# tmbdev/clstm

Hardware: AMD Instinct MI355X
Metric: text-line images/sec (fwd+bwd+CTC), 100-unit BiLSTM H=48 T~200 (higher is better)
Workload: dtype f32 (operand-exact split): forward, recurrences, CTC, decode in f32 arithmetic; the backward weight-gradient / softmax-backward products take their f32 operands split EXACTLY into three bf16 terms each (x1 + x2 + x3 = x) and sum the six bf16-MFMA products of weight >= 2^-16 in f32 -- what is dropped

## Files before the change

clstm_amd/csrc/dbgopt.h:

```cpp
#pragma once
#include <cstdlib>
#include <cstring>
#include <map>
#include <stdexcept>
#include <string>

namespace clstm {
struct DbgOptDef { const char* name; int dflt; };
inline constexpr DbgOptDef DBG_OPTS[] = {
    {"gemm_stag", 2},
    {"bwd_c32", 1},
    {"rec_x3", 1},
    {"pack_tiles", 1},
    {"fuse_wx", 1},
    {"gemm_b16mc", 1},
    {"dw_x3", 1},
    {"gemm_x3", 1},
    {"split_terms", 3},
    {"xd_prologue", 2},
    {"fwd_mfma", 1},
    {"bwd_mfma", 1},
    {"bwd_mfma_fused", 1},
    {"ctc_float", 0},
    {"peer_two_phase", 1},
};
inline const DbgOptDef* dbg_opt_def(const char* name) {
  for (const DbgOptDef& o : DBG_OPTS)
    if (strcmp(o.name, name) == 0) return &o;
  return nullptr;
}
inline std::map<std::string, int>& dbg_opts() {
  static std::map<std::string, int> m = [] {
    std::map<std::string, int> r;
    const char* e = getenv("CLSTM_DEBUG");
    if (e) {
      std::string s(e);
      size_t i = 0;
      while (i < s.size()) {
        size_t j = s.find(',', i);
        if (j == std::string::npos) j = s.size();
        const std::string kv = s.substr(i, j - i);
        const size_t eq = kv.find('=');
        if (!kv.empty()) {
          const std::string name = kv.substr(0, eq);
          if (eq == std::string::npos || !dbg_opt_def(name.c_str()))
            throw std::runtime_error("CLSTM_DEBUG: unknown option '" + name + "' (clstm_amd/csrc/dbgopt.h lists them as name=value)");
          r[name] = atoi(kv.c_str() + eq + 1);
        }
        i = j + 1;
      }
    }
    return r;
  }();
  return m;
}
inline int dbg_opt(const char* name) {
  const DbgOptDef* d = dbg_opt_def(name);
  if (!d) throw std::logic_error(std::string("internal: option '") + name + "' is not in DBG_OPTS");
  const auto& m = dbg_opts();
  const auto it = m.find(name);
  return it == m.end() ? d->dflt : it->second;
}
}
```

clstm_amd/csrc/devintrin.h:

```cpp
#pragma once

#ifdef CLSTM_HIP_EMU
#include "hip_emu.h"
#else
#include <hip/hip_runtime.h>
#include <hip/hip_ext.h>
#include <vector>

typedef float f32x4 __attribute__((ext_vector_type(4)));
typedef float f32x2 __attribute__((ext_vector_type(2)));
typedef unsigned u32x2 __attribute__((ext_vector_type(2)));

#define DEVFN __device__ __forceinline__
#define DEVMFN __device__ __forceinline__

template <int CTRL>
DEVFN float dpp_mov(float x) {
  const int xi = __builtin_bit_cast(int, x);
  return __builtin_bit_cast(float, __builtin_amdgcn_update_dpp(xi, xi, CTRL, 0xF, 0xF, false));
}
template <int CTRL>
DEVFN float dpp_perm(float x) {
  return __builtin_bit_cast(float, __builtin_amdgcn_update_dpp(0, __builtin_bit_cast(int, x), CTRL, 0xF, 0xF, true));
}
// ... 119 lines not shown
typedef unsigned u32x4 __attribute__((ext_vector_type(4)));
DEVFN u32x2 lds_read_tr16(const unsigned short* p) {
  return __builtin_bit_cast(u32x2, __builtin_amdgcn_ds_read_tr16_b64_v4i16((i16x4 __attribute__((address_space(3)))*)p));
}
typedef unsigned LdsAddr;
DEVFN LdsAddr lds_addr(const void* p) { return (unsigned)(size_t)(const __attribute__((address_space(3))) void*)p; }
DEVFN LdsAddr lds_addr_add(LdsAddr a, int bytes) { return a + (unsigned)bytes; }
template <int OFF>
DEVFN u32x2 lds_read_tr16_raw(LdsAddr addr) {
  u32x2 r;
  asm volatile("ds_read_b64_tr_b16 %0, %1 offset:%2" : "=v"(r) : "v"(addr), "n"(OFF));
  return r;
}
DEVFN u16x8 join_u16x8(u32x2 a, u32x2 b) {
  u32x4 v;
  v[0] = a[0]; v[1] = a[1]; v[2] = b[0]; v[3] = b[1];
  return __builtin_bit_cast(u16x8, v);
}

DEVFN int wave_uniform(int x) { return __builtin_amdgcn_readfirstlane(x); }
DEVFN long long dev_clock() { return (long long)__builtin_readcyclecounter(); }
DEVFN long long wall_clock() { return (long long)__builtin_amdgcn_s_memrealtime(); }
DEVFN float fast_exp(float x) { return __expf(x); }
DEVFN float fast_exp2(float x) { return __builtin_amdgcn_exp2f(x); }
DEVFN float fast_rcp(float x) { return __builtin_amdgcn_rcpf(x); }
DEVFN float fast_log2(float x) { return __builtin_amdgcn_logf(x); }

struct BufF32 { __amdgpu_buffer_rsrc_t r; };
constexpr unsigned BUF_OOB = 0xFFFFFFF0u;
constexpr unsigned BUF_OOB_BASE = 0x80000000u;
DEVFN BufF32 make_buf(const float* base, size_t bytes) {
  BufF32 b;
  b.r = __builtin_amdgcn_make_buffer_rsrc((void*)base, 0, (int)(bytes > 0x7FFFFFF0ull ? 0x7FFFFFF0ull : bytes), 0x00020000);
  return b;
}
DEVFN float buf_load(BufF32 b, unsigned byte_off) {
  return __builtin_bit_cast(float, __builtin_amdgcn_raw_buffer_load_b32(b.r, byte_off, 0, 0));
}
typedef int i32x4 __attribute__((ext_vector_type(4)));
typedef int i32x2 __attribute__((ext_vector_type(2)));
DEVFN f32x4 buf_load4(BufF32 b, unsigned byte_off) {
  return __builtin_bit_cast(f32x4, __builtin_amdgcn_raw_buffer_load_b128(b.r, byte_off, 0, 0));
}
DEVFN void buf_store(BufF32 b, unsigned byte_off, float v) {
  __builtin_amdgcn_raw_buffer_store_b32(__builtin_bit_cast(int, v), b.r, byte_off, 0, 0);
}
DEVFN void lds_dma16(BufF32 b, unsigned byte_off, void* lds_wave_base) {
  __builtin_amdgcn_raw_ptr_buffer_load_lds(b.r, (__attribute__((address_space(3))) void*)lds_wave_base, 16, byte_off, 0, 0, 0);
}
DEVFN void lds_dma4(BufF32 b, unsigned byte_off, void* lds_wave_base) {
  __builtin_amdgcn_raw_ptr_buffer_load_lds(b.r, (__attribute__((address_space(3))) void*)lds_wave_base, 4, byte_off, 0, 0, 0);
}
template <int N> DEVFN void wait_vmcnt() { asm volatile("s_waitcnt vmcnt(%0)" ::"n"(N) : "memory"); }
DEVFN void wait_lgkmcnt0() { asm volatile("s_waitcnt lgkmcnt(0)" ::: "memory"); }
DEVFN void wg_barrier() { __builtin_amdgcn_s_barrier(); }
DEVFN void wave_lds_fence() { __builtin_amdgcn_fence(__ATOMIC_ACQ_REL, "wavefront"); }
DEVFN float buf_load_s(BufF32 b, unsigned lane_off, unsigned uniform_off) {
  return __builtin_bit_cast(float, __builtin_amdgcn_raw_buffer_load_b32(b.r, lane_off, uniform_off, 0));
}
DEVFN void buf_store_s(BufF32 b, unsigned lane_off, unsigned uniform_off, float v) {
  __builtin_amdgcn_raw_buffer_store_b32(__builtin_bit_cast(int, v), b.r, lane_off, uniform_off, 0);
}
DEVFN void buf_store4(BufF32 b, unsigned byte_off, f32x4 v) {
  __builtin_amdgcn_raw_buffer_store_b128(__builtin_bit_cast(i32x4, v), b.r, byte_off, 0, 0);
}
DEVFN void buf_store_u32(BufF32 b, unsigned byte_off, unsigned v) { __builtin_amdgcn_raw_buffer_store_b32((int)v, b.r, byte_off, 0, 0); }
DEVFN void buf_store_u32x2_s(BufF32 b, unsigned lane_off, unsigned uniform_off, u32x2 v) {
  __builtin_amdgcn_raw_buffer_store_b64(__builtin_bit_cast(i32x2, v), b.r, lane_off, uniform_off, 0);
}
DEVFN void buf_store_u32_s(BufF32 b, unsigned lane_off, unsigned uniform_off, unsigned v) {
  __builtin_amdgcn_raw_buffer_store_b32((int)v, b.r, lane_off, uniform_off, 0);
}
DEVFN float max_f32(float x, float y) {
  float r;
  asm("v_max_f32 %0, %1, %2" : "=v"(r) : "v"(x), "v"(y));
  return r;
}

DEVFN f32x4 buf_load4_dev(BufF32 b, unsigned byte_off) {
  return __builtin_bit_cast(f32x4, __builtin_amdgcn_raw_buffer_load_b128(b.r, byte_off, 0, 16));
}
#define COMPILER_MEMORY_BARRIER() asm volatile("" ::: "memory")
DEVFN void buf_store_wt(BufF32 b, unsigned byte_off, float v) {
  __builtin_amdgcn_raw_buffer_store_b32(__builtin_bit_cast(int, v), b.r, byte_off, 0, 17);
}
DEVFN f32x4 buf_load4_wt(BufF32 b, unsigned byte_off) {
  return __builtin_bit_cast(f32x4, __builtin_amdgcn_raw_buffer_load_b128(b.r, byte_off, 0, 17));
}
DEVFN float buf_load_wt(BufF32 b, unsigned byte_off) {
  return __builtin_bit_cast(float, __builtin_amdgcn_raw_buffer_load_b32(b.r, byte_off, 0, 17));
}
DEVFN void buf_store4_wt(BufF32 b, unsigned byte_off, f32x4 v) {
  __builtin_amdgcn_raw_buffer_store_b128(__builtin_bit_cast(i32x4, v), b.r, byte_off, 0, 17);
}
DEVFN int load_i32_wt(const int* p) { return __hip_atomic_load(p, __ATOMIC_RELAXED, __HIP_MEMORY_SCOPE_SYSTEM); }
DEVFN void store_i32_wt(int* p, int v) { __hip_atomic_store(p, v, __ATOMIC_RELAXED, __HIP_MEMORY_SCOPE_SYSTEM); }
DEVFN void atomic_add_i32(int* p, int v) { atomicAdd(p, v); }
DEVFN int atomic_fetch_add_i32(int* p, int v) { return atomicAdd(p, v); }
DEVFN int hw_xcc_id() { unsigned x; asm volatile("s_getreg_b32 %0, hwreg(HW_REG_XCC_ID)" : "=s"(x)); return (int)(x & 0xF); }
DEVFN void sleep_some() { __builtin_amdgcn_s_sleep(16); }
DEVFN void poll_pause() { __builtin_amdgcn_s_sleep(1); }
DEVFN void sleep_iterations(int n) {
  n = n > 40 ? 40 : n;
  for (int i = 0; i < n; i++) __builtin_amdgcn_s_sleep(13);
}
DEVFN int wave_max_i(int x) {
#pragma unroll
  for (int m = 32; m >= 1; m >>= 1) { const int y = __shfl_xor(x, m, 64); x = y > x ? y : x; }
  return x;
}
DEVFN void drain_vmem() { asm volatile("s_waitcnt vmcnt(0)" ::: "memory"); }
DEVFN unsigned mad_u24(unsigned a, unsigned b, unsigned c) { return __umul24(a, b) + c; }
constexpr int GRID_WATCHDOG_SPINS = 1 << 21;
struct ClstmLaunchEvents { hipEvent_t a, b; };
inline thread_local std::vector<ClstmLaunchEvents>* clstm_launch_sink = nullptr;
inline thread_local std::vector<ClstmLaunchEvents> clstm_event_pool;
inline ClstmLaunchEvents clstm_launch_events() {
  ClstmLaunchEvents e{};
  if (!clstm_event_pool.empty()) { e = clstm_event_pool.back(); clstm_event_pool.pop_back(); }
  else { (void)hipEventCreate(&e.a); (void)hipEventCreate(&e.b); }
  clstm_launch_sink->push_back(e);
  return e;
}
#define CLSTM_LAUNCH_COOP(kernel, grid, block, smem, stream, argstruct)                                  \
  do {                                                                                                   \
    void* coop_args_[] = {(void*)&(argstruct)};                                                          \
    ClstmLaunchEvents ev_{};                                                                             \
    if (clstm_launch_sink) { ev_ = clstm_launch_events(); HIPCHECK(hipEventRecord(ev_.a, (hipStream_t)(stream))); } \
    HIPCHECK(hipLaunchCooperativeKernel((const void*)(kernel), grid, block, coop_args_, smem, (hipStream_t)(stream))); \
    if (ev_.b) HIPCHECK(hipEventRecord(ev_.b, (hipStream_t)(stream)));                                   \
  } while (0)

#define KEEP_ALIVE(x) asm volatile("" ::"v"(x))
#define SCHED_FENCE() __builtin_amdgcn_sched_barrier(0)
#define OPAQUE(x) asm volatile("" : "+v"(x))
#define KEEP_ALIVE2(x) asm volatile("" ::"v"(x))

template <typename T>
DEVFN T* dyn_smem() {
  extern __shared__ __attribute__((aligned(16))) char clstm_dyn_smem_[];
  return reinterpret_cast<T*>(clstm_dyn_smem_);
}

#define CLSTM_LAUNCH(kernel, grid, block, smem, stream, ...)                                                       \
  do {                                                                                                             \
    if (__builtin_expect(clstm_launch_sink != nullptr, 0)) {                                                       \
      const ClstmLaunchEvents ev_ = clstm_launch_events();                                                         \
      hipExtLaunchKernelGGL(kernel, grid, block, smem, (hipStream_t)(stream), ev_.a, ev_.b, 0, __VA_ARGS__);       \
    } else hipLaunchKernelGGL(kernel, grid, block, smem, (hipStream_t)(stream), __VA_ARGS__);                      \
  } while (0)
#endif

DEVFN bool dev_err_set(const int* err) { return err && (err[0] | err[1] | err[2] | err[3] | err[6] | err[7]) != 0; }
DEVFN bool f32_finite(float x) { return (__builtin_bit_cast(unsigned, x) & 0x7f800000u) != 0x7f800000u; }
DEVFN void raise_nonfinite(int* nanflag, int step_no) { if (*nanflag == 0) *nanflag = step_no; }


constexpr int PROG_STRIDE = 32;

constexpr int STAG_NA = 64, STAG_KA = 16;
__host__ __device__ inline constexpr bool stag_on(int nk4) { return nk4 >= 5; }
__host__ __device__ inline int stag_fwd_k(int q, int kk, int ku) { return kk < STAG_KA ? STAG_KA * q + kk : STAG_NA + (ku - STAG_KA) * q + (kk - STAG_KA); }
__host__ __device__ inline int stag_fwd_slot(int cell, int ku, int qs) {
  return cell < STAG_NA ? (cell / STAG_KA) * qs + (cell % STAG_KA)
                        : ((cell - STAG_NA) / (ku - STAG_KA)) * qs + STAG_KA + (cell - STAG_NA) % (ku - STAG_KA);
}

DEVFN float tanh_dev(float x) {
  const float xc = fminf(fmaxf(x, -15.0f), 15.0f);
  const float e = fast_exp(2.0f * xc);
  const float big = (e - 1.0f) * fast_rcp(e + 1.0f);
  const float small = xc - xc * xc * xc * (1.0f / 3.0f);
  return fabsf(xc) < 0.01f ? small : big;
}

DEVFN float sigmoid_dev(float x) { return fast_rcp(1.0f + fast_exp(-x)); }

DEVFN float gate_act(float x, bool is_tanh) {
  const float ax = fabsf(x);
  const unsigned mask = is_tanh ? 0x7FFFFFFFu : 0xFFFFFFFFu;
  const float scale = is_tanh ? -2.0f * 1.44269504088896341f : -1.44269504088896341f;
  const float e = fast_exp2(__builtin_bit_cast(float, __builtin_bit_cast(unsigned, x) & mask) * scale);
  const float r = fast_rcp(1.0f + e);
  const float s = ax * ax;
  const float p = fmaf(s, fmaf(s, fmaf(s, fmaf(s, fmaf(s, -1382.0f / 155925.0f, 62.0f / 2835.0f), -17.0f / 315.0f), 2.0f / 15.0f), -1.0f / 3.0f), 1.0f);
  const float th = copysignf(ax < 0.35f ? ax * p : (1.0f - e) * r, x);
  return is_tanh ? th : r;
}

constexpr float ACT_SIG_SCALE = -1.44269504088896341f, ACT_TANH_SCALE = -2.0f * 1.44269504088896341f;
DEVFN float act_affine(float x, float scale, float A, float B) {
  const float r = fast_rcp(1.0f + fast_exp2(x * scale));
  return fmaf(r, A, B);
}
DEVFN float tanh_fast(float x) { return act_affine(x, ACT_TANH_SCALE, 2.0f, -1.0f); }
```

clstm_amd/csrc/gemm_dw.h:

```cpp
#pragma once
#include <type_traits>
#include "gemm_bf16.h"

namespace clstm {

struct DwSlab {
  int tile_begin, ntiles;
  int need_it;
  int dir;
  int out_z;
  int pad[3];
};

struct XdArgs {
  GemmOperand A;
  GemmOperand B;
  float* out; int ld;
  int K;
  int* ready; int ready0;
};

struct GemmDwArgs {
  const float* S; long long sdir; int lds; long long s_elems;
  const float* D; int M; int no4; long long d_elems;
  const int* ktab;
  int ntiles_max;
  const DwSlab* slabs;
  int nslabs;
  const int* prog;
  const int* line_off;
  int bs, prog_base, ndir;
  float* partial;
  int R, Cn;
  unsigned gx, gy;
  int* timeouts;
  int* minprog;
  int tcap;
  int* done;
  int done_target;
  long long* trace;
  int trace_base;
  const float* xS; int xlds; long long xs_elems;
  const float* xD; int xM; long long xd_elems;
  const int* xtab; const DwSlab* xslabs; int xnslabs;
  float* xpartial; int xR, xCn; unsigned xgx, xgy;
  int x3;
  int terms;
  XdArgs xd;
};

constexpr int DW_PF = 3;
constexpr int DW_STAB_MAX = 256;
constexpr int dw_img_floats(int nt) { return nt <= 2 ? 8192 : 2 * 2 * nt * 64 * 32 / 2; }
constexpr int dw_smem_floats(int nt) { return dw_img_floats(nt) + 2 * DW_STAB_MAX; }
static_assert(8192 >= GEMM_BT * GEMM_LDO, "epilogue tile");

constexpr int DW_WATCHDOG_POLLS = 1 << 16;

DEVFN void gemm_dw_monitor(const GemmDwArgs& a) {
  if (threadIdx.x >= 64) return;
  const int lane = threadIdx.x & 63;
  int polls = 0;
  for (;;) {
    int all = 0x3fffffff;
    int pv[2][4];
#pragma unroll
    for (int dir = 0; dir < 2; dir++)
#pragma unroll
      for (int j = 0; j < 4; j++) {
        const int b = lane + 64 * j;
        pv[dir][j] = dir < a.ndir && b < a.bs ? load_i32_wt(a.prog + ((size_t)dir * a.bs + b) * PROG_STRIDE) : 0;
      }
    for (int dir = 0; dir < a.ndir; dir++) {
      int m = 0x3fffffff;
      for (int b = lane, j = 0; b < a.bs; b += 64, j++) {
        const int T = a.line_off[b + 1] - a.line_off[b];
        const int p = (j < 4 ? pv[dir][j] : load_i32_wt(a.prog + ((size_t)dir * a.bs + b) * PROG_STRIDE)) - a.prog_base;
        const int v = p >= T ? 0x3fffffff : (p < 0 ? 0 : p);
        m = v < m ? v : m;
      }
      m = -wave_max_i(-m);
      if (lane == 0) store_i32_wt(a.minprog + dir * PROG_STRIDE, a.prog_base + (m > a.tcap ? a.tcap : m));
      all = m < all ? m : all;
    }
    if (all >= 0x3fffffff) break;
    if (++polls > (DW_WATCHDOG_POLLS << 4)) {
      if (lane == 0) {
        atomic_add_i32(a.timeouts, 1);
        for (int dir = 0; dir < a.ndir; dir++) store_i32_wt(a.minprog + dir * PROG_STRIDE, a.prog_base + a.tcap);
      }
      break;
    }
  }
}

DEVFN void gemm_dw_wait(const GemmDwArgs& a, const int dir, const int need_it) {
  const int wave = wave_uniform(threadIdx.x >> 6);
  if (wave == 0) {
    const int need = need_it < a.tcap ? need_it : a.tcap;
    const bool all = a.done && need_it >= a.tcap - 32;
    int polls = 0;
    for (;;) {
      int have;
      if (all) have = (int)((unsigned)wave_uniform(load_i32_wt(a.done)) - (unsigned)a.done_target) >= 0 ? need : need - 1;
      else have = wave_uniform(load_i32_wt(a.minprog + dir * PROG_STRIDE) - a.prog_base);
      if (have >= need) break;
      if (++polls > (DW_WATCHDOG_POLLS << 4)) {
        if ((threadIdx.x & 63) == 0) atomic_add_i32(a.timeouts, 1);
        break;
      }
      const int deficit = need - (have < 0 ? 0 : have);
      sleep_iterations(deficit > 12 ? 6 : 1);
    }
  }
  __syncthreads();
}

DEVFN void gemm_dw_item(const GemmDwArgs& a, float* smem, const unsigned si, const unsigned tile) {
  float* As = smem;
  float* Bs = smem + GEMM_BK * GEMM_LD;
  const int tid = threadIdx.x;
  const int lane = tid & 63, wave = wave_uniform(tid >> 6);
  const int wm = wave >> 1, wn = wave & 1;
  const DwSlab sl = a.slabs[si];
  const int r0 = (int)(tile / a.gx) * GEMM_BT, c0 = (int)(tile % a.gx) * GEMM_BT;
  const int dir = sl.dir;
  gemm_dw_wait(a, dir, sl.need_it);

  const int a_mn = (tid & 15) * 4, a_k = tid >> 4;
  const BufF32 abuf = make_buf(a.S + (size_t)dir * a.sdir, (size_t)(a.s_elems - (long long)dir * a.sdir) * 4);
  const BufF32 bbuf = make_buf(a.D, (size_t)a.d_elems * 4);
  const unsigned a_col = (unsigned)(r0 + a_mn), b_col = (unsigned)(dir * a.no4 + c0 + a_mn);
  const int* tab = a.ktab + (size_t)dir * a.ntiles_max * 2;
  const int tend = sl.tile_begin + sl.ntiles;

  auto load_tile = [&](int t, f32x4& ra, f32x4& rb, int& cnt) {
    const bool live = t < tend;
    const int tt = live ? t : sl.tile_begin;
    const int f0 = tab[2 * tt];
    cnt = live ? tab[2 * tt + 1] : 0;
    const bool row = a_k < cnt;
    const unsigned f = (unsigned)(f0 + a_k);
    ra = buf_load4(abuf, row ? (f * (unsigned)a.lds + a_col) * 4u : BUF_OOB);
    rb = buf_load4_wt(bbuf, row ? (f * (unsigned)a.M + b_col) * 4u : BUF_OOB);
  };

  f32x4 acc[2][2];
#pragma unroll
  for (int i = 0; i < 2; i++)
#pragma unroll
    for (int j = 0; j < 2; j++)
#pragma unroll
      for (int q = 0; q < 4; q++) acc[i][j][q] = 0.0f;

  f32x4 ra[GEMM_PF], rb[GEMM_PF];
  int cnt[GEMM_PF];
#pragma unroll
  for (int p = 0; p < GEMM_PF; p++) {
    load_tile(sl.tile_begin + p, ra[p], rb[p], cnt[p]);
    SCHED_FENCE();
  }
  const int fk = lane >> 4, fi = lane & 15;
  for (int tb = sl.tile_begin; tb < tend; tb += GEMM_PF) {
#pragma unroll
    for (int p = 0; p < GEMM_PF; p++) {
      const bool row = a_k < cnt[p];
#pragma unroll
      for (int i = 0; i < 4; i++) {
        ra[p][i] = row ? ra[p][i] : 0.0f;
        rb[p][i] = row ? rb[p][i] : 0.0f;
      }
      *reinterpret_cast<f32x4*>(&As[a_k * GEMM_LD + a_mn]) = ra[p];
      *reinterpret_cast<f32x4*>(&Bs[a_k * GEMM_LD + a_mn]) = rb[p];
      __syncthreads();
      load_tile(tb + p + GEMM_PF, ra[p], rb[p], cnt[p]);
      SCHED_FENCE();
#pragma unroll
      for (int kk = 0; kk < GEMM_BK; kk += 4) {
        float af[2], bf[2];
#pragma unroll
        for (int i = 0; i < 2; i++) {
          af[i] = As[(kk + fk) * GEMM_LD + wm * 32 + i * 16 + fi];
          bf[i] = Bs[(kk + fk) * GEMM_LD + wn * 32 + i * 16 + fi];
        }
#pragma unroll
        for (int i = 0; i < 2; i++)
#pragma unroll
          for (int j = 0; j < 2; j++) acc[i][j] = mfma16x16x4(af[i], bf[j], acc[i][j]);
      }
      __syncthreads();
    }
  }
#pragma unroll
  for (int i = 0; i < 2; i++)
#pragma unroll
    for (int j = 0; j < 2; j++)
#pragma unroll
      for (int q = 0; q < 4; q++)
        smem[(wm * 32 + i * 16 + (lane >> 4) * 4 + q) * GEMM_LDO + wn * 32 + j * 16 + (lane & 15)] = acc[i][j][q];
  __syncthreads();
  float* out = a.partial + (size_t)sl.out_z * a.R * a.Cn;
  const bool v4 = (a.Cn & 3) == 0 && ((size_t)a.partial & 15) == 0;
#pragma unroll
  for (int it = 0; it < 4; it++) {
    const int rl = it * 16 + (tid >> 4), cl = (tid & 15) * 4;
    const int r = r0 + rl, c = c0 + cl;
    const f32x4 v = *reinterpret_cast<const f32x4*>(&smem[rl * GEMM_LDO + cl]);
    if (r < a.R) {
      if (v4 && c + 3 < a.Cn) *reinterpret_cast<f32x4*>(out + (size_t)r * a.Cn + c) = v;
      else
        for (int e = 0; e < 4; e++)
          if (c + e < a.Cn) out[(size_t)r * a.Cn + c + e] = v[e];
    }
  }
}
template <int NT>
DEVFN void gemm_dw_item_x3(const GemmDwArgs& a, float* smem, const unsigned si, const unsigned tile, const bool extra = false) {
  constexpr int IMG = 64 * 32;
  constexpr int BUFH = 2 * NT * IMG;
  unsigned short* img = reinterpret_cast<unsigned short*>(smem);
  const int tid = threadIdx.x;
  const int lane = tid & 63, wave = wave_uniform(tid >> 6);
  const int wm = wave >> 1, wn = wave & 1;
  const DwSlab sl = extra ? a.xslabs[si] : a.slabs[si];
  const unsigned pgx = extra ? a.xgx : a.gx;
  const int pR = extra ? a.xR : a.R, pCn = extra ? a.xCn : a.Cn;
  const int r0 = (int)(tile / pgx) * GEMM_BT, c0 = (int)(tile % pgx) * GEMM_BT;
  const int dir = sl.dir;
  const long long t_start = a.trace ? wall_clock() : 0;
  const int* tab = extra ? a.xtab : a.ktab + (size_t)dir * a.ntiles_max * 2;
  int* stab = reinterpret_cast<int*>(smem + dw_img_floats(NT));
  for (int i = tid; i < 2 * sl.ntiles && i < 2 * DW_STAB_MAX; i += 256) stab[i] = tab[2 * sl.tile_begin + i];
  if (sl.need_it > 0) gemm_dw_wait(a, dir, sl.need_it);
  else __syncthreads();
  const long long t_ready = a.trace ? wall_clock() : 0;

  const bool isB = wave >= 2;
  const int s_mn = (wave & 1) * 32 + (lane & 7) * 4, s_kg = lane >> 3;
  const BufF32 abuf = extra ? make_buf(a.xS, (size_t)a.xs_elems * 4)
                            : make_buf(a.S + (size_t)dir * a.sdir, (size_t)(a.s_elems - (long long)dir * a.sdir) * 4);
  const BufF32 bbuf = extra ? make_buf(a.xD, (size_t)a.xd_elems * 4) : make_buf(a.D, (size_t)a.d_elems * 4);
  const unsigned col = isB ? (unsigned)((extra ? 0 : dir * a.no4) + c0 + s_mn) : (unsigned)(r0 + s_mn);
  const unsigned ldrow = isB ? (unsigned)(extra ? a.xM : a.M) : (unsigned)(extra ? a.xlds : a.lds);
  const int tend = sl.tile_begin + sl.ntiles;
  const int e_half = s_kg >> 2, kk0 = (s_kg & 3) * 4;

  auto load_block = [&](auto role, int t, f32x4 (&r)[4]) {
    constexpr bool ROLE_B = decltype(role)::value;
    const int te = t + e_half;
    const bool live = te < tend;
    const int tt = live ? te : sl.tile_begin;
    const int f0 = stab[2 * (tt - sl.tile_begin)];
    const int cn = stab[2 * (tt - sl.tile_begin) + 1];
    const int cnt = live ? cn : 0;
#pragma unroll
    for (int j = 0; j < 4; j++) {
      const unsigned off = kk0 + j < cnt ? ((unsigned)(f0 + kk0 + j) * ldrow + col) * 4u : BUF_OOB;
      if constexpr (ROLE_B) r[j] = buf_load4_wt(bbuf, off);
      else r[j] = buf_load4(abuf, off);
    }
  };
  unsigned short* const my_img = img + (isB ? NT * IMG : 0);
  int wofs[4];
#pragma unroll
  for (int i = 0; i < 4; i++) wofs[i] = (s_mn + i) * 32 + ((((s_kg >> 1) ^ gb2_sw(s_mn + i)) << 3) | ((s_kg & 1) << 2));
  auto stage = [&](int buf, const f32x4 (&r)[4]) {
    unsigned short* d = my_img + buf * BUFH;
#pragma unroll
    for (int i = 0; i < 4; i++) {
      float e[4] = {r[0][i], r[1][i], r[2][i], r[3][i]};
#pragma unroll
      for (int t = 0; t < NT; t++) {
        u32x2 h;
        h[0] = bf16_pack2(e[0], e[1]);
        h[1] = bf16_pack2(e[2], e[3]);
        *reinterpret_cast<u32x2*>(d + t * IMG + wofs[i]) = h;
        if (t + 1 < NT) {
          e[0] -= __builtin_bit_cast(float, h[0] << 16); e[1] -= __builtin_bit_cast(float, h[0] & 0xffff0000u);
          e[2] -= __builtin_bit_cast(float, h[1] << 16); e[3] -= __builtin_bit_cast(float, h[1] & 0xffff0000u);
        }
      }
    }
  };

  f32x4 acc[2][2];
#pragma unroll
  for (int i = 0; i < 2; i++)
#pragma unroll
    for (int j = 0; j < 2; j++)
#pragma unroll
      for (int q = 0; q < 4; q++) acc[i][j][q] = 0.0f;

  const int fk = lane >> 4, fi = lane & 15;
  const int fofs = fi * 32 + ((fk ^ gb2_sw(fi)) << 3);
  auto run = [&](auto role) {
  f32x4 rr[DW_PF][4];
#pragma unroll
  for (int p = 0; p < DW_PF; p++) {
    load_block(role, sl.tile_begin + 2 * p, rr[p]);
    SCHED_FENCE();
  }
  stage(0, rr[0]);
  load_block(role, sl.tile_begin + 2 * DW_PF, rr[0]);
  SCHED_FENCE();
  __syncthreads();
  int cur = 0;
  for (int tb = sl.tile_begin; tb < tend; tb += 2 * DW_PF) {
#pragma unroll
    for (int p = 0; p < DW_PF; p++) {
      const int pn = p + 1 == DW_PF ? 0 : p + 1;
      stage(cur ^ 1, rr[pn]);
      load_block(role, tb + 2 * (p + 1 + DW_PF), rr[pn]);
      SCHED_FENCE();
      const unsigned short* b0 = img + cur * BUFH;
      u16x8 at[NT][2], bt[NT][2];
#pragma unroll
      for (int t = 0; t < NT; t++)
#pragma unroll
        for (int i = 0; i < 2; i++) {
          at[t][i] = *reinterpret_cast<const u16x8*>(b0 + t * IMG + (wm * 32 + i * 16) * 32 + fofs);
          bt[t][i] = *reinterpret_cast<const u16x8*>(b0 + (NT + t) * IMG + (wn * 32 + i * 16) * 32 + fofs);
        }
#pragma unroll
      for (int w = NT - 1; w >= 0; w--)
#pragma unroll
        for (int ta = 0; ta <= w; ta++)
#pragma unroll
          for (int i = 0; i < 2; i++)
#pragma unroll
            for (int j = 0; j < 2; j++) acc[i][j] = mfma16x16x32_bf16(at[ta][i], bt[w - ta][j], acc[i][j]);
      __syncthreads();
      cur ^= 1;
    }
  }
  };
  if (isB) run(std::true_type{}); else run(std::false_type{});
#pragma unroll
  for (int i = 0; i < 2; i++)
#pragma unroll
    for (int j = 0; j < 2; j++)
#pragma unroll
      for (int q = 0; q < 4; q++)
        smem[(wm * 32 + i * 16 + (lane >> 4) * 4 + q) * GEMM_LDO + wn * 32 + j * 16 + (lane & 15)] = acc[i][j][q];
  __syncthreads();
  float* out = (extra ? a.xpartial : a.partial) + (size_t)sl.out_z * pR * pCn;
  const bool v4 = (pCn & 3) == 0 && ((size_t)out & 15) == 0;
#pragma unroll
  for (int it = 0; it < 4; it++) {
    const int rl = it * 16 + (tid >> 4), cl = (tid & 15) * 4;
    const int r = r0 + rl, c = c0 + cl;
    const f32x4 v = *reinterpret_cast<const f32x4*>(&smem[rl * GEMM_LDO + cl]);
    if (r < pR) {
      if (v4 && c + 3 < pCn) *reinterpret_cast<f32x4*>(out + (size_t)r * pCn + c) = v;
      else
        for (int e = 0; e < 4; e++)
          if (c + e < pCn) out[(size_t)r * pCn + c + e] = v[e];
    }
  }
  if (a.trace && tid == 0 && !extra) {
    long long* tr = a.trace + ((size_t)a.trace_base + si * (a.gx * a.gy) + tile) * 4;
    tr[0] = t_start; tr[1] = t_ready; tr[2] = wall_clock(); tr[3] = sl.need_it;
  }
}

template <int NT>
DEVFN void gemm_dw_body(const GemmDwArgs& a, float* smem, unsigned block) {
  constexpr bool X3 = NT != 0;
  if (block == 0) { gemm_dw_monitor(a); return; }
  block -= 1;
  const unsigned nextra = X3 ? (unsigned)a.xnslabs * a.xgx * a.xgy : 0u;
  if constexpr (X3) {
    if (block < nextra) { gemm_dw_item_x3<NT>(a, smem, block / (a.xgx * a.xgy), block % (a.xgx * a.xgy), true); return; }
  }
  block -= nextra;
  const unsigned tiles = a.gx * a.gy;
  const unsigned xcd = block & 7u, idx = block >> 3;
  const unsigned si = (idx / tiles) * 8u + xcd;
  if (si >= (unsigned)a.nslabs) return;
  if constexpr (X3) gemm_dw_item_x3<NT>(a, smem, si, idx % tiles);
  else gemm_dw_item(a, smem, si, idx % tiles);
}
template <int NT>
__global__ __launch_bounds__(256) void gemm_dw_kernel(GemmDwArgs a) {
  __shared__ __attribute__((aligned(16))) float smem[dw_smem_floats(NT)];
  gemm_dw_body<NT>(a, smem, blockIdx.x);
}

}
```

clstm_amd/csrc/lstm_bwd_dw.h:

```cpp
#pragma once
#include "gemm_dw.h"
#include "lstm_seq.h"
#include "lstm_xd_prologue.h"

namespace clstm {

constexpr int DW_FUSED_STAB_ENTRIES = 1024;
static_assert(DW_FUSED_STAB_ENTRIES >= DW_STAB_MAX, "the items' k-tile table fits");
static_assert(xd_smem_floats(2) <= dw_img_floats(2) && xd_smem_floats(3) <= dw_img_floats(3), "the recurrence role's x.d prologue stages in the items' carve");

template <int NK4, int KU, int NT>
__global__ __launch_bounds__(64 * NK4) CLSTM_TWO_WAVES_PER_SIMD void lstm_bwd_dw_kernel(LstmSeqArgs a, GemmDwArgs g, int nrec) {
  __shared__ __attribute__((aligned(16))) float gsm[dw_img_floats(NT) + 2 * DW_FUSED_STAB_ENTRIES];
  if ((int)blockIdx.x < nrec) {
#ifndef CLSTM_HIP_EMU
    __builtin_amdgcn_s_setprio(3);
#endif
    const long long t0 = g.trace ? wall_clock() : 0;
    const int bl = (int)blockIdx.x % a.bs;
    const int b = a.order ? a.order[bl] : bl, dir = (int)blockIdx.x / a.bs;
    bool producers = false;
    if constexpr (NT >= 2) {
      if (g.xd.A.p) {
        producers = g.xd.ready != nullptr;
        if (producers) xd_own_round<NT, xd_maxu(NK4)>(gsm, g.xd, a.line_off, b, dir, a.no);
        else xd_prologue<NT, xd_maxu(NK4)>(gsm, g.xd, a.line_off, b, dir, a.no);
      }
    }
    const long long t1 = g.trace ? wall_clock() : 0;
    if constexpr (NT >= 2) {
      if (producers) lstm_bwd_body<NK4, KU, true>(a, b, dir, g.xd.ready + ((size_t)dir * a.bs + b) * PROG_STRIDE, g.xd.ready0);
      else lstm_bwd_body<NK4, KU>(a, b, dir);
    } else lstm_bwd_body<NK4, KU>(a, b, dir);
    if (g.done && threadIdx.x == 0) atomic_add_i32(g.done, 1);
    if (g.trace && threadIdx.x == 0) { g.trace[blockIdx.x * 4] = t0; g.trace[blockIdx.x * 4 + 1] = t1; g.trace[blockIdx.x * 4 + 2] = wall_clock(); }
  } else {
    unsigned blk = blockIdx.x - (unsigned)nrec;
    if constexpr (NT >= 2) {
      if (g.xd.ready) {
        if (blk >= 1u && blk <= (unsigned)nrec) { xd_item<NT, xd_maxu(NK4)>(gsm, g.xd, a.line_off, a.order, a.bs, (int)blk - 1, a.no); return; }
        if (blk > (unsigned)nrec) blk -= (unsigned)nrec;
      }
    }
    if (threadIdx.x >= 256) return;
    gemm_dw_body<NT>(g, gsm, blk);
  }
}

}
```

clstm_amd/csrc/net.inc:

```
struct Layer {
  int ni, no, nk4, nthreads;
  bool wide = false;
  int kpf = 0, kpb = 0;
  int kp16f = 0, kp16b = 0, rowsf = 0, rowsb = 0;
  bool bwd_exact = false;
  long long nwf = 0, nwb = 0;
  PackDesc pd;
  float *Wt = nullptr, *bias = nullptr, *Rf = nullptr, *Rb = nullptr, *Rwf = nullptr, *Rwb = nullptr;
  float* Wk = nullptr;
  int wk_kp = 0, wk_njp = 0;
  DevBuf<float> dCc;
  DevBuf<unsigned short> Wmf;
  DevBuf<float> mf_scale;
  DevBuf<unsigned> mf_xmax;
  long long mf_epoch = -1;
  DevBuf<unsigned short> Wmfb;
  long long mfb_epoch = -1;
  DevBuf<int> pack_tab;
  DevBuf<int> pack_inv;
  int pack_inv_state = 0;
  unsigned short *Rbf = nullptr, *Rbb = nullptr;
  DevBuf<unsigned short> R2b, D2;
  bool r2b_ready = false;
  DevBuf<unsigned short> Hb, Db;
  DevBuf<float> Rf32;
  long long* moff = nullptr;
  DevBuf<float> G, C, H, D, dH, S;
  DevBuf<unsigned short> Hbf;
  DevBuf<unsigned short> WtbT;
  bool fwd_persistent = false;
  DevBuf<unsigned short> Sbf;
  bool sbf_ready = false;
  bool sbf_x_external = false;
  long long sbf_one_key = -1;
  bool d_f32_valid = true;
  bool sx_valid = true;
  bool h_f32_valid = true;
  bool sh_valid = true;
  DevBuf<unsigned short> Dbf;
  DevBuf<float> dbias;
  DevBuf<float> partial;
  DevBuf<unsigned short> Wtb;
  int lds = 0;
  int wt_slack = 32;
  int ldh = 0, hofs = 4;
  float* hrow() const { return H.p + hofs; }
  float* srow() const { return H.p + hofs - 1; }
};

enum class BwdFamily { Overlapped, Wide, Narrow };
struct BwdPlan {
  BwdFamily family;
  bool bwd_persistent;
  bool dw_from_bf16;
  bool dw_bias_out;
  bool x3_big;
  int dw_rows, ns;
};

struct Minibatch {
  const int* T; int bs; const float* x; const int* labels; const int* L;
  bool given() const { return T && x && labels && L && bs > 0; }
};
static long long batch_frames(const int* T_h, int nb) {
  long long n = 0;
  for (int b = 0; b < nb; b++) { REQUIRE(T_h[b] >= 0, "negative line length"); n += T_h[b]; }
  REQUIRE(n > 0, "batch has no frames");
  return n;
}
struct HostTicket { int* word = nullptr; int id = 0; };
struct StepPlan {
  bool fuse = false;
  bool peer = false;
  bool defer_last = false;
  HostTicket ticket;
};
struct DeferredReduce { bool armed = false; ReduceDesc gates, extra; float* gdst = nullptr; UpdateFuse uf; size_t work = 0; hipStream_t q = nullptr; };
struct PassLeft {
  bool update_applied = false;
  bool packs_follow_update = false;
  bool peer_pending = false;
  DeferredReduce deferred;
  HostTicket ticket;
};

struct Net {
  clstm_net_desc desc;
  int ndir;
  std::vector<Layer> L;
  int sm_ni = 0;
  long long sm_off = 0;
  int nparams = 0;
  float *v = nullptr, *d = nullptr, *g = nullptr;
  bool own_v = false, own_d = false, own_g = false;
  float lr = 1e-4f, mom = 0.9f, gclip = 100.0f;
  bool packed_dirty = true;
  long long params_epoch = 0;
  bool bf16_gemm = false;
  bool bf16_rec = false;
  bool want_dx0 = false;
  int bs = 0, tmax = 0;
  bool src0_ready = false;
  long long N = 0;
  std::vector<int> line_off_h;
  DevBuf<int> line_off;
  std::vector<int> order_h;
  PinnedRing ring;
  const int* lo_stage = nullptr;
  bool lo_pending = false;
  void flush_line_off() {
    if (!lo_pending) return;
    hipStream_t s = stream();
    HIPCHECK(hipMemcpyAsync(line_off.p, lo_stage, (2 * bs + 1) * sizeof(int), hipMemcpyHostToDevice, s));
    ring.commit(s);
    lo_pending = false;
  }
  DevBuf<float> X, Z, Dz, dX0, partial, partial_sm, aligned, tmp;
  DevBuf<unsigned short> xbf;
  ReduceDesc sm_red{};
  DevBuf<long long> lstm_prof;
  StepGraphCache step_graphs;
  XcdSync coop_sync;
  Timing timing;
  static const int PROG_WORDS = 2 * PROG_LINES * PROG_STRIDE;
  int overlap = getenv("CLSTM_OVERLAP") ? atoi(getenv("CLSTM_OVERLAP")) : 1;
  unsigned dw_done_total = 0;
  DevBuf<long long> dw_trace;
  DevBuf<int> xd_ready;
  DevBuf<int> dw_ktab, dw_slabs, dw_queue;
  std::vector<int> dw_key;
  DevBuf<int> dwx_tab;
  long long dwx_N = -1;
  int dwx_nslabs = 0, dwx_entries = 0;
  int dw_nslabs = 0, dw_slabs_per_dir = 0, dw_ntiles_max = 0;
  int prog_base = 1024;
  long long dw_launches = 0;
  Comm* comm = nullptr;
  struct HostFeed {
    hipStream_t cs = nullptr;
    hipEvent_t copied[2] = {};
    DevBuf<float> xin[2];
    PinnedBuf<char> pin[2];
    int* step_done = nullptr;
    long long steps = 0;
    bool ready = false;
    const float* stage(const float* x_h, size_t nfloats, HostTicket& ticket) {
      if (!ready) {
        ready = true;
        HIPCHECK(hipStreamCreateWithFlags(&cs, hipStreamNonBlocking));
        for (int i = 0; i < 2; i++) HIPCHECK(hipEventCreateWithFlags(&copied[i], hipEventDisableTiming));
        HIPCHECK(hipHostMalloc((void**)&step_done, 64));
        *step_done = 0;
      }
      const long long k = steps + 1;
      const int slot = (int)(k & 1);
      {
        const auto t0 = std::chrono::steady_clock::now();
        int spins = 0;
        while (k > 2 && (int)((unsigned)(k - 2) - (unsigned)__atomic_load_n(step_done, __ATOMIC_ACQUIRE)) > 0) {
          sched_yield();
          if ((++spins & 1023) == 0 && std::chrono::steady_clock::now() - t0 > std::chrono::seconds(2)) {
            HIPCHECK(hipStreamSynchronize(g_stream));
            check_device_errors();
            break;
          }
        }
      }
      const size_t bytes = nfloats * sizeof(float);
      xin[slot].reserve(nfloats + 64);
      const void* src = x_h;
#ifndef CLSTM_HIP_EMU
      hipPointerAttribute_t attr;
      const bool pinned = hipPointerGetAttributes(&attr, x_h) == hipSuccess && attr.type == hipMemoryTypeHost;
      if (!pinned) {
        (void)hipGetLastError();
        pin[slot].reserve(bytes);
        memcpy(pin[slot].p, x_h, bytes);
        src = pin[slot].p;
      }
#endif
      HIPCHECK(hipMemcpyAsync(xin[slot].p, src, bytes, hipMemcpyHostToDevice, cs));
      HIPCHECK(hipEventRecord(copied[slot], cs));
      HIPCHECK(hipStreamWaitEvent(g_stream, copied[slot], 0));
      ticket = HostTicket{step_done, (int)(unsigned)k};
      return xin[slot].p;
    }
    void commit() { steps++; }
  } hf;
  float* W1k = nullptr;
  int w1k_kps = 0;
  DevBuf<int> fw_items, fw_flags;
  std::vector<int> fw_key;
  int fw_npitems = 0, fw_ncitems = 0, fw_chunks = 0;
  int fw_epoch = 0, fw_prog_base = 1024;
  long long fw_launches = 0;

  hipStream_t stream() const { return g_stream; }
  bool geom_predict = false, nosave = false, in_predict = false;
  size_t fixed_bytes = 0;
  void dev_malloc(void** q, size_t bytes) { HIPCHECK(hipMalloc(q, bytes)); fixed_bytes += bytes; }

  static bool l_is_only_layer(const clstm_net_desc& ds) { return ds.nlayers == 1; }
  int* pack_table(Layer& y) {
    if (!y.pack_tab.p) {
      const PackFused pf = pack_fused_desc(y);
      const size_t n = pack_count(y);
      y.pack_tab.reserve(n);
      CLSTM_LAUNCH(k_pack_index, dim3(nblocks(n)), dim3(256), 0, stream(), y.pack_tab.p, y.pd, pf);
      check_launch();
    }
    return y.pack_tab.p;
  }
  static constexpr int PACK_KD = 4;
  size_t pack_count(const Layer& y) const {
    const PackFused pf = pack_fused_desc(y);
    return (size_t)(1 + y.ni) * ndir * 4 * y.no + 2 * ((size_t)ndir * 4 * 4 * y.nk4 * y.nthreads) +
           (pf.Wk ? (size_t)ndir * pf.njp * 16 * pf.kp + (size_t)96 * pf.kps : 0);
  }
  bool pack_inverse(Layer& y) {
    if (y.pack_inv_state) return y.pack_inv_state > 0;
    const int* tab = pack_table(y);
    const size_t n = pack_count(y);
    std::vector<int> t(n);
    HIPCHECK(hipMemcpyAsync(t.data(), tab, n * sizeof(int), hipMemcpyDeviceToHost, stream()));
    HIPCHECK(hipStreamSynchronize(stream()));
    std::vector<int> inv((size_t)nparams * PACK_KD, -1), cnt(nparams, 0);
    y.pack_inv_state = 1;
    for (size_t e = 0; e < n && y.pack_inv_state > 0; e++) {
      const int si = t[e];
      if (si < 0) continue;
      if (si >= nparams || cnt[si] >= PACK_KD) { y.pack_inv_state = -1; break; }
      inv[(size_t)si * PACK_KD + cnt[si]++] = (int)e;
    }
    if (y.pack_inv_state < 0) return false;
    y.pack_inv.reserve(inv.size());
    HIPCHECK(hipMemcpyAsync(y.pack_inv.p, inv.data(), inv.size() * sizeof(int), hipMemcpyHostToDevice, stream()));
    HIPCHECK(hipStreamSynchronize(stream()));
    return true;
  }
  PackFused pack_fused_desc(const Layer& y) const {
    PackFused f{};
    if (y.Wk) { f.Wk = y.Wk; f.kp = y.wk_kp; f.njp = y.wk_njp; f.W1k = W1k; f.kps = w1k_kps; f.nc = desc.nclasses; f.sm_k = sm_ni; f.sm_off = sm_off; }
    return f;
  }
  void build(const clstm_net_desc& ds, float* pv, float* pd, float* pg) {
    desc = ds;
    REQUIRE(ds.nlayers >= 1 && ds.nlayers <= CLSTM_MAX_LAYERS, "nlayers out of range");
    REQUIRE(ds.ninput > 0 && ds.nclasses >= 2, "bad ninput/nclasses (Softmax requires no>=2, clstm.cc:399)");
    ndir = ds.unidirectional ? 1 : 2;
    static const int blockidx[4] = {2, 1, 3, 0};
    long long off = 0;
    int ni = ds.ninput;
    L.resize(ds.nlayers);
    for (int l = 0; l < ds.nlayers; l++) {
      Layer& y = L[l];
      y.ni = ni;
      y.no = ds.nhidden[l];
      REQUIRE(y.no > 0, "nhidden must be positive");
      const NarrowClass k = narrow_class(y.no);
      const bool force_wide = getenv("CLSTM_FORCE_WIDE") && atoi(getenv("CLSTM_FORCE_WIDE")) != 0;
      y.wide = !k.nk4 || force_wide;
      y.nk4 = y.wide ? 1 : k.nk4;
      y.nthreads = y.wide ? 64 : 64 * k.waves;
      REQUIRE(y.wide || y.nthreads * xd_maxu(y.nk4) >= XD_UNITS, "internal: a workgroup of this class does not cover a staging round of the x.d prologue");
      y.kp16f = wide_kp16_fwd(y.no); y.kp16b = wide_kp16_bwd(y.no);
      y.rowsf = (y.no + 3) / 4 * 16; y.rowsb = (y.no + 15) / 16 * 16;
      y.bwd_exact = y.kp16b == 4 * y.no;
      y.lds = ((1 + y.ni + y.no + 15) / 16) * 16;
      y.ldh = ((y.hofs + ndir * y.no + 15) / 16) * 16;
      const long long blk = (long long)y.no * (1 + y.ni + y.no);
      y.pd.ni = y.ni; y.pd.no = y.no; y.pd.ndir = ndir; y.pd.nk4 = y.nk4; y.pd.nthreads = y.wide ? 0 : y.nthreads; y.pd.ku = y.wide ? 4 : k.ku;
      for (int dir = 0; dir < ndir; dir++) {
        for (int s = 0; s < 4; s++) y.pd.p_off[dir][s] = off + blockidx[s] * blk;
        off += 4 * blk;
      }
      if (ndir == 1) for (int s = 0; s < 4; s++) y.pd.p_off[1][s] = y.pd.p_off[0][s];
      ni = ndir * y.no;
    }
    sm_ni = ni;
    sm_off = off;
    off += (long long)ds.nclasses * (1 + sm_ni);
    nparams = (int)off;
    auto own = [&](float*& dst, float* given, bool& flag) {
      if (given) { dst = given; flag = false; }
      else {
        dev_malloc((void**)&dst, (size_t)nparams * sizeof(float));
        zero_fill(dst, (size_t)nparams * sizeof(float));
        flag = true;
// ... 507 lines not shown
        timing.begin("lstm_fwd", s);
        launch_lstm(true, y.nk4, y.pd.ku, a, bs, y.nthreads, s, save);
        count_moves(np.moves);
        if (save) y.h_f32_valid = y.sh_valid = true;
        timing.end(s);
      }
      if (save && !y.sbf_ready) ensure_source_x(l);
    }
    forward_softmax();
  }
  void forward_softmax() {
    hipStream_t s = stream();
    const int nc = desc.nclasses;
    const float* W1 = v + sm_off;
    if (nc <= SMX_COLS) {
      timing.begin("gemm_softmax", s);
      softmax_fwd(s, gemm_kc(L.back().hrow(), L.back().ldh, N), W1, (long long)nc * (1 + sm_ni), Z.p, (int)N, nc, sm_ni, fwd_nanflag(), step_no() + 1);
      timing.end(s);
      check_launch();
    } else {
      timing.begin("gemm_softmax", s);
      if (bf16_gemm && gemm_x3_on && gemm_bf16_big((int)N, nc))
        gemm_x3_big<GEMM_KC, GEMM_MC>(s, gemm_kc(L.back().hrow(), L.back().ldh, N, 32), gemm_mc(W1 + nc, nc, sm_ni, 0),
                                      StoreBias{Z.p, nc, W1}, (int)N, nc, sm_ni);
      else
      gemm_f32<GEMM_KC, GEMM_MC>(s, gemm_kc(L.back().hrow(), L.back().ldh, N), gemm_mc(W1 + nc, nc, sm_ni, 0),
                                 StoreBias{Z.p, nc, W1}, (int)N, nc, sm_ni);
      timing.end(s);
      check_launch();
      timing.begin("softmax_norm", s);
      CLSTM_LAUNCH(k_softmax_norm, dim3((unsigned)((N + 3) / 4)), dim3(256), 0, s, Z.p, nc, (size_t)N, fwd_nanflag(), step_no() + 1);
      timing.end(s);
      check_launch();
    }
  }

  void predict() {
    REQUIRE(N > 0, "set_batch first");
    RoctxRange range_("clstm:predict");
    struct Guard { bool& f; Guard(bool& x) : f(x) { f = true; } ~Guard() { f = false; } } guard_(in_predict);
    if (!geom_predict) { forward(); return; }
    nosave = true;
    src0_ready = false;
    for (auto& y : L) { y.sx_valid = y.sh_valid = false; y.h_f32_valid = true; y.sbf_ready = false; y.fwd_persistent = false; }
    forward_pass(false);
  }

  void build_fwd_items() {
    if (fw_key == line_off_h && fw_ncitems > 0) return;
    fw_chunks = (tmax + 15) / 16;
    std::vector<int> items;
    for (int c = 1; c < fw_chunks; c += FWD_FT)
      for (int i = 0; i < bs; i++) {
        const int b = order_h[i], T = line_off_h[b + 1] - line_off_h[b];
        if (T > 16 * c)
          for (int dir = 0; dir < ndir; dir++) { items.push_back(b << 13 | dir << 12 | c); items.push_back(line_off_h[b]); items.push_back(T); items.push_back(0); }
      }
    fw_npitems = (int)items.size() / 4;
    std::vector<std::pair<int, int>> cons;
    for (int b = 0; b < bs; b++) {
      const int T = line_off_h[b + 1] - line_off_h[b];
      for (int blk = 0; 16 * blk < T; blk++)
        cons.push_back({std::max(std::min(16 * blk + 16, T), ndir > 1 ? T - 16 * blk : 0), b << 12 | blk});
    }
    std::stable_sort(cons.begin(), cons.end(), [](const std::pair<int, int>& x, const std::pair<int, int>& y) { return x.first < y.first; });
    fw_ncitems = (int)cons.size();
    for (auto& c : cons) items.push_back(c.second);
    fw_items.reserve(items.size() + 8);
    fw_flags.reserve((size_t)ndir * bs * fw_chunks + 8);
    hipStream_t s = stream();
    int* stage = (int*)ring.acquire(items.size() * sizeof(int));
    memcpy(stage, items.data(), items.size() * sizeof(int));
    HIPCHECK(hipMemcpyAsync(fw_items.p, stage, items.size() * sizeof(int), hipMemcpyHostToDevice, s));
    ring.commit(s);
    fw_key = line_off_h;
  }
  void forward_fused(const NarrowPlan& np, bool save) {
    hipStream_t s = stream();
    Layer& y = L[0];
    build_fwd_items();
    if (++fw_epoch > (1 << 30)) fw_epoch = 1;
    fw_prog_base += tmax + 64;
    if (fw_prog_base > (1 << 30)) fw_prog_base = 1024;
    fw_launches++;
    count_moves(np.moves);
    FwdFusedKernelArgs k{};
    LstmSeqArgs& a = k.a;
    a = seq_args(y, true, save);
    a.prog_off = (long long)y.H.cap - 64 - PROG_WORDS;
    REQUIRE(a.prog_off >= (long long)N * y.ldh + 16, "internal: progress words overlap the output rows");
    a.prog_base = fw_prog_base;
    a.gflag = fw_flags.p; a.gchunks = fw_chunks; a.gepoch = fw_epoch; a.timeouts = dev_err_words() + 2;
    FwdFusedArgs& h = k.h;
    h.X = layer_input(0); h.ldx = layer_input_ld(0); h.x_elems = (long long)N * h.ldx + 32;
    h.Wk = y.Wk; h.kp = y.wk_kp; h.njp = y.wk_njp; h.bias = y.bias;
    h.pitems = fw_items.p; h.npitems = fw_npitems; h.gflag = fw_flags.p;
    h.W1k = W1k; h.kps = w1k_kps; h.sm_k = sm_ni; h.b1 = v + sm_off; h.Z = Z.p; h.nc = desc.nclasses;
    h.citems = fw_items.p + 4 * fw_npitems; h.ncitems = fw_ncitems;
    h.nanflag = fwd_nanflag(); h.step_no = step_no() + 1;
    h.prog = (const int*)(y.H.p + a.prog_off);
    h.nrec = bs * ndir; h.npb = fw_npitems;
    const unsigned nblk = (unsigned)(h.nrec + h.npb + fw_ncitems);
    if (save) { y.sx_valid = src0_ready; ensure_source_x(0); }
    static const char* trace_path = getenv("CLSTM_FW_TRACE");
    const size_t trace_rows = (size_t)h.nrec + fw_npitems + fw_ncitems;
    if (trace_path) { dw_trace.reserve(trace_rows * 4); HIPCHECK(hipMemsetAsync(dw_trace.p, 0, trace_rows * 4 * sizeof(long long), s)); h.trace = dw_trace.p; }
    timing.begin("lstm_fwd", s);
    launch_lstm_fwd_fused(y.nk4, y.pd.ku, k, nblk, y.nthreads, s, save);
    timing.end(s);
    if (trace_path)
      dump_trace(trace_path, dw_trace.p, trace_rows, s,
                 "# %d recurrence rows (start - end -), %d producer items (start - done chunk), %d consumer items (start ready done ready_iteration); 100 MHz ticks\n",
                 h.nrec, fw_npitems, fw_ncitems);
  }

  bool dw_x3 = dbg_opt("dw_x3") != 0;
  int split_terms = dbg_opt("split_terms");
  bool gemm_x3_on = dbg_opt("gemm_x3") != 0;
  bool strict_f32 = false;
  bool rec_x3() const {
    if (bf16_gemm || bf16_rec || !gemm_x3_on) return false;
    return dbg_opt("rec_x3") != 0;
  }
  int clamp_split(long long want) const { return (int)std::max(1LL, std::min({want, (long long)(N + 63) / 64, 64LL})); }
  int pick_split_mc(int R, int Cn, int nbatch) const {
    const int th = gemm_mc_tile_rows(R);
    const long long tiles = (long long)((R + th - 1) / th) * ((Cn + 255) / 256) * nbatch;
    return clamp_split(device_cu_count() / tiles);
  }
  int pick_split(int R, int Cn, int nbatch = 1, int tile = GEMM_BT) const {
    const long long tiles = (long long)((R + tile - 1) / tile) * ((Cn + tile - 1) / tile) * nbatch;
    const long long target = tile == GEMM_BT ? 640 : 480;
    long long want = (target + tiles - 1) / tiles;
    if (tile == 256) want = device_cu_count() / tiles;
    return clamp_split(want);
  }

  XdArgs xd_args() const {
    const Layer& top = L.back();
    const int nc = desc.nclasses;
    return XdArgs{gemm_kc(Dz.p, nc, N), gemm_kc(v + sm_off + nc, nc, sm_ni, 0), top.dH.p, sm_ni, nc, nullptr, 0};
  }
  static int dw_bf16_rows(const Layer& y, int R, int Cn) { return y.bwd_exact && gemm_bf16_big(R - 1, Cn) ? R - 1 : R; }
  static constexpr int DW_CHUNK = 16, DW_TAIL_PARTS = 4, DW_TAIL_CHUNKS = 2;
  void build_dw_tables() {
    if (dw_key == line_off_h && dw_nslabs > 0) return;
    std::vector<int> cb;
    for (int done = DW_CHUNK; done < tmax; done += DW_CHUNK) cb.push_back(done);
    cb.push_back(tmax);
    const int tiles_per_slab = std::min(DW_STAB_MAX, std::max(8, (int)((N / 16 + 15) / 16)));
    std::vector<std::vector<int>> tab(ndir);
    struct Sl { int tb, nt, need, dir, chunk, part; };
    std::vector<std::vector<Sl>> sl(ndir);
    for (int dir = 0; dir < ndir; dir++) {
      int cs = 0;
      for (size_t c = 0; c < cb.size(); c++) {
        const int ce = cb[c];
        const int t0 = (int)tab[dir].size() / 2;
        for (int b = 0; b < bs; b++) {
          const int off = line_off_h[b], T = line_off_h[b + 1] - off;
          if (T <= cs) continue;
          const int e = std::min(ce, T);
          const int f_lo = dir == 0 ? T - e : cs, f_hi = dir == 0 ? T - cs : e;
          for (int f = f_lo; f < f_hi; f += 16) { tab[dir].push_back(off + f); tab[dir].push_back(std::min(16, f_hi - f)); }
        }
        const int nt = (int)tab[dir].size() / 2 - t0;
        int parts = std::max(1, (nt + tiles_per_slab - 1) / tiles_per_slab);
        if (c + DW_TAIL_CHUNKS >= cb.size()) parts = std::max(parts, std::min(DW_TAIL_PARTS, std::max(1, nt / 2)));
        for (int p = 0; p < parts; p++) {
          const int a0 = t0 + (int)((long long)nt * p / parts), a1 = t0 + (int)((long long)nt * (p + 1) / parts);
          REQUIRE(a1 - a0 <= DW_STAB_MAX, "internal: weight-gradient slab longer than its LDS table");
          sl[dir].push_back(Sl{a0, a1 - a0, ce, dir, (int)c, p});
        }
        cs = ce;
      }
    }
    dw_slabs_per_dir = (int)sl[0].size();
    for (int dir = 1; dir < ndir; dir++) REQUIRE((int)sl[dir].size() == dw_slabs_per_dir, "internal: asymmetric slab lists");
    dw_ntiles_max = 0;
    for (int dir = 0; dir < ndir; dir++) dw_ntiles_max = std::max(dw_ntiles_max, (int)tab[dir].size() / 2);
    std::vector<DwSlab> slabs;
    for (int i = 0; i < dw_slabs_per_dir; i++)
      for (int dir = 0; dir < ndir; dir++) {
        const Sl& x = sl[dir][i];
        slabs.push_back(DwSlab{x.tb, x.nt, x.need, dir, dir * dw_slabs_per_dir + i, {0, 0, 0}});
      }
    dw_nslabs = (int)slabs.size();
    const size_t nk = (size_t)ndir * dw_ntiles_max * 2, nsw = slabs.size() * sizeof(DwSlab) / sizeof(int);
    dw_ktab.reserve(nk + 8);
    dw_slabs.reserve(nsw + 8);
    hipStream_t s = stream();
    int* stage = (int*)ring.acquire((nk + nsw) * sizeof(int));
    for (int dir = 0; dir < ndir; dir++) {
      std::fill(stage + (size_t)dir * dw_ntiles_max * 2, stage + (size_t)(dir + 1) * dw_ntiles_max * 2, 0);
      std::copy(tab[dir].begin(), tab[dir].end(), stage + (size_t)dir * dw_ntiles_max * 2);
    }
    memcpy(stage + nk, slabs.data(), nsw * sizeof(int));
    HIPCHECK(hipMemcpyAsync(dw_ktab.p, stage, nk * sizeof(int), hipMemcpyHostToDevice, s));
    HIPCHECK(hipMemcpyAsync(dw_slabs.p, stage + nk, nsw * sizeof(int), hipMemcpyHostToDevice, s));
    ring.commit(s);
    dw_key = line_off_h;
  }
  void backward_layer_overlapped(Layer& y, const NarrowPlan& np, LstmSeqArgs a, int R, int Cn) {
    hipStream_t s = stream();
    build_dw_tables();
    const int M = ndir * 4 * y.no;
    const long long prog_off = (long long)y.D.cap - 64 - PROG_WORDS;
    REQUIRE(prog_off >= (long long)N * M, "internal: progress words overlap the deltas");
    prog_base += tmax + 64;
    dw_launches++;
    const bool prog_base_wrapped = prog_base > (1 << 30);
    if (prog_base_wrapped) prog_base = 1024;
    a.prog_off = prog_off;
    a.prog_base = prog_base;
    DevBuf<float>& partial = layer_partial(y);
    partial.reserve((size_t)ndir * dw_slabs_per_dir * R * Cn);
    GemmDwArgs g{};
    g.S = y.S.p; g.sdir = (long long)N * y.lds; g.lds = y.lds; g.s_elems = (long long)N * ndir * y.lds + 3;
    g.D = y.D.p; g.M = M; g.no4 = 4 * y.no; g.d_elems = (long long)N * M + 3;
    g.ktab = dw_ktab.p; g.ntiles_max = dw_ntiles_max; g.slabs = (const DwSlab*)dw_slabs.p; g.nslabs = dw_nslabs;
    g.prog = (const int*)(y.D.p + prog_off); g.line_off = line_off.p; g.bs = bs; g.prog_base = prog_base;
    g.partial = partial.p; g.R = R; g.Cn = Cn;
    g.gx = (unsigned)((Cn + GEMM_BT - 1) / GEMM_BT); g.gy = (unsigned)((R + GEMM_BT - 1) / GEMM_BT);
    g.timeouts = dev_err_words() + 1;
    if (!dw_queue.p) dw_queue.reserve(5 * PROG_STRIDE);
    g.ndir = ndir;
    g.minprog = dw_queue.p + PROG_STRIDE;
    g.tcap = tmax + 32;
    g.done = nullptr; g.done_target = 0;
    g.x3 = dw_x3;
    g.terms = split_terms;
    unsigned nextra = 0;
    if (np.xd) g.xd = xd_args();
    if (np.xd == 2) {
      const size_t nw = (size_t)ndir * bs * PROG_STRIDE;
      if (nw > xd_ready.cap || prog_base_wrapped) {
        xd_ready.reserve(nw);
        HIPCHECK(hipMemsetAsync(xd_ready.p, 0, xd_ready.cap * sizeof(int), s));
      }
      g.xd.ready = xd_ready.p; g.xd.ready0 = prog_base;
      a.timeouts = g.timeouts;
    }
    if (np.dwx) {
      const int xR = 1 + sm_ni, xCn = desc.nclasses;
      g.xS = y.srow(); g.xlds = y.ldh; g.xs_elems = (long long)N * y.ldh + 3;
      g.xD = Dz.p; g.xM = xCn; g.xd_elems = (long long)N * xCn + 3;
      g.xtab = dwx_tab.p; g.xslabs = (const DwSlab*)(dwx_tab.p + 2 * dwx_entries); g.xnslabs = dwx_nslabs;
      g.xpartial = partial_sm.p; g.xR = xR; g.xCn = xCn;
      g.xgx = (unsigned)((xCn + GEMM_BT - 1) / GEMM_BT); g.xgy = (unsigned)((xR + GEMM_BT - 1) / GEMM_BT);
      nextra = (unsigned)dwx_nslabs * g.xgx * g.xgy;
    }
    static const char* trace_path = getenv("CLSTM_DW_TRACE");
    const size_t trace_rows = (size_t)bs * ndir + (size_t)((dw_nslabs + 7) / 8) * 8 * g.gx * g.gy + 8;
    if (trace_path) { dw_trace.reserve(trace_rows * 4); g.trace = dw_trace.p; g.trace_base = bs * ndir; }
    const unsigned nblk = 1u + (np.xd == 2 ? (unsigned)(bs * ndir) : 0u) + nextra + (unsigned)((dw_nslabs + 7) / 8) * 8u * g.gx * g.gy;
    timing.begin("lstm_bwd", s);
    if (np.bwd == NB_MFMA_DW) launch_mfma_bwd(y, a, s, &g, nblk);
    else if (np.bwd == NB_BWD_DW) {
      g.done = g.minprog + 2 * PROG_STRIDE;
      dw_done_total += (unsigned)(bs * ndir);
      g.done_target = (int)dw_done_total;
      launch_lstm_bwd_dw(y.nk4, y.pd.ku, a, g, np.terms, bs * ndir, nblk, y.nthreads, s);
    } else launch_bwd_narrow(y, np, a, s, &g.xd);
    timing.end(s);
    if (np.bwd == NB_BWD_DW && trace_path)
      dump_trace(trace_path, dw_trace.p, trace_rows, s,
                 "# rows 0..%d: recurrence workgroups (start, x.d prologue returned, end); then one row per (slab, tile) item: start ready done need_it; 100 MHz ticks\n", bs * ndir - 1);
    if (np.bwd == NB_MFMA_DW || np.bwd == NB_BWD_DW) return;
    timing.begin("gemm_gates_dw", s);
    launch_gemm_dw(g, np.terms, nblk, s);
    timing.end(s);
  }

  void build_dwx_table() {
    if (dwx_N == N) return;
    hipStream_t s = stream();
    dwx_entries = (int)((N + 15) / 16);
    const int eps = std::min(DW_STAB_MAX, std::max(32, (dwx_entries + 63) / 64));
    dwx_nslabs = (dwx_entries + eps - 1) / eps;
    const size_t nsw = (size_t)dwx_nslabs * sizeof(DwSlab) / sizeof(int);
    dwx_tab.reserve((size_t)2 * dwx_entries + nsw + 8);
    int* stage = (int*)ring.acquire(((size_t)2 * dwx_entries + nsw) * sizeof(int));
    for (int e = 0; e < dwx_entries; e++) { stage[2 * e] = 16 * e; stage[2 * e + 1] = (int)std::min<long long>(16, N - 16LL * e); }
    DwSlab* sl = (DwSlab*)(stage + 2 * dwx_entries);
    for (int i = 0; i < dwx_nslabs; i++) sl[i] = DwSlab{eps * i, std::min(eps, dwx_entries - eps * i), 0, 0, i, {0, 0, 0}};
    for (int i = 0; i < dwx_nslabs; i++) REQUIRE(sl[i].ntiles <= DW_STAB_MAX, "internal: weight-gradient slab longer than its LDS table");
    HIPCHECK(hipMemcpyAsync(dwx_tab.p, stage, ((size_t)2 * dwx_entries + nsw) * sizeof(int), hipMemcpyHostToDevice, s));
    ring.commit(s);
    dwx_N = N;
  }
  struct ReduceTarget { const StepPlan& plan; float* gdst; PassLeft& left; };
  PassLeft backward(const StepPlan& plan = StepPlan{}) {
    REQUIRE(N > 0, "set_batch first");
    PassLeft left;
    left.ticket = plan.ticket;
    const ReduceTarget rt{plan, plan.peer ? comm->peer.slot_ptr(comm->peer.seq + 1) : g, left};
    nbackward++;
    RoctxRange range_("clstm:backward");
    pending_red.clear();
    flush_line_off();
    repack();
    hipStream_t s = stream();
    NarrowPlan np[CLSTM_MAX_LAYERS];
    for (int l = 0; l < (int)L.size(); l++) np[l] = backward_plan_narrow(l);
    backward_softmax(np[L.size() - 1]);
    for (int l = (int)L.size() - 1; l >= 0; l--) {
      const BwdFamily fam = L[l].wide ? BwdFamily::Wide : np[l].overlapped ? BwdFamily::Overlapped : BwdFamily::Narrow;
      const bool bwd_persistent = backward_recurrence(l, fam, np[l]);
      const BwdPlan p = backward_plan(L[l], fam, bwd_persistent);
      if (!p.dw_from_bf16) { ensure_source(l); ensure_delta_f32(l); }
      if (!backward_weight_gradient(l, p, rt)) backward_input_deltas(l, p);
    }
    if (!pending_red.empty()) {
      timing.begin("reduce_scatter", s);
      for (size_t i = 0; i < pending_red.size(); i++) reduce_layer(pending_red[i].gates, pending_red[i].extra, i + 1 == pending_red.size(), rt);
      pending_red.clear();
      timing.end(s);
      check_launch();
    }
    return left;
  }
  void backward_softmax(const NarrowPlan& top_plan) {
    hipStream_t s = stream();
    Layer& top = L.back();
    const int nc = desc.nclasses, R = 1 + sm_ni, Cn = nc;
    const float* W1 = v + sm_off;
    const bool sm_big = bf16_gemm && gemm_x3_on && gemm_bf16_big(R, Cn) && gemm_bf16_big((int)N, sm_ni);
    int ns = sm_big ? pick_split(R, Cn, 1, GB2_BT) : pick_split(R, Cn);
    if (top_plan.dwx) { build_dwx_table(); ns = dwx_nslabs; }
    partial_sm.reserve((size_t)ns * R * Cn);
    const GemmOperand Wk = gemm_kc(W1 + nc, nc, sm_ni, 0);
    const StorePartial wd_store{partial_sm.p, R, Cn};
    const StorePlain xd_store{top.dH.p, sm_ni};
    const bool launches = !top_plan.xd;
    if (launches) timing.begin("gemm_softmax_dw_dx", s);
    if (top_plan.dwx) {
      if (launches) gemm_x3<GEMM_KC, GEMM_KC>(s, gemm_kc(Dz.p, nc, N), Wk, xd_store, (int)N, sm_ni, nc, 1, 1, split_terms);
    } else if (sm_big) {
      gemm_x3_big<GEMM_MC, GEMM_MC>(s, gemm_mc(top.srow(), top.ldh, N, 32), gemm_mc(Dz.p, nc, N, 32), wd_store, R, Cn, (int)N, ns);
      gemm_x3_big<GEMM_KC, GEMM_KC>(s, gemm_kc(Dz.p, nc, N, 32), Wk, xd_store, (int)N, sm_ni, nc);
    } else {
      const GemmProblem wd = gemm_problem(gemm_mc(top.srow(), top.ldh, N), gemm_mc(Dz.p, nc, N), R, Cn, (int)N, ns);
      const GemmProblem xd = gemm_problem(gemm_kc(Dz.p, nc, N), Wk, (int)N, sm_ni, nc);
      if (gemm_x3_on) gemm_x3_pair<GEMM_MC, GEMM_MC, StorePartial, GEMM_KC, GEMM_KC, StorePlain>(s, wd, wd_store, xd, xd_store, split_terms);
      else gemm_f32_pair<GEMM_MC, GEMM_MC, StorePartial, GEMM_KC, GEMM_KC, StorePlain>(s, wd, wd_store, xd, xd_store);
    }
    if (launches) timing.end(s);
    sm_red = ReduceDesc{partial_sm.p, nullptr, (long long)sm_off, ns, 1, R, Cn, nc};
    check_launch();
  }
  bool backward_recurrence(int l, BwdFamily fam, const NarrowPlan& np) {
    Layer& y = L[l];
    hipStream_t s = stream();
    const LstmSeqArgs a = seq_args(y, false);
    if (fam == BwdFamily::Overlapped) {
      backward_layer_overlapped(y, np, a, 1 + y.ni + y.no, 4 * y.no);
      count_moves(np.moves);
      return false;
    }
    timing.begin("lstm_bwd", s);
    WideRan ran = WideRan::Nothing;
    int skipped_d = 0;
    if (fam == BwdFamily::Wide) {
      const LstmWideArgs w = wide_args(y, false);
      ran = launch_lstm_wide(wide_plan(wide_shape(y, false)), w, coop_sync, step_graphs, s);
      skipped_d = w.skip_d;
    } else { launch_bwd_narrow(y, np, a, s); count_moves(np.moves); }
    timing.end(s);
    const bool persistent = ran == WideRan::Persistent;
    y.d_f32_valid = !(persistent && bf16_rec && skipped_d);
    return persistent;
  }
  BwdPlan backward_plan(const Layer& y, BwdFamily fam, bool bwd_persistent) const {
    const int R = 1 + y.ni + y.no, Cn = 4 * y.no;
    BwdPlan p{};
    p.family = fam; p.bwd_persistent = bwd_persistent;
    p.dw_from_bf16 = bf16_gemm && bf16_rec && bwd_persistent && y.sbf_ready && y.Dbf.p && gemm_bf16_big(R, Cn);
    p.dw_rows = p.dw_from_bf16 ? dw_bf16_rows(y, R, Cn) : R;
    p.dw_bias_out = p.dw_rows < R;
    REQUIRE(!p.dw_bias_out || y.dbias.p, "internal: bias row left out of the weight-gradient product without the recurrence's per-line sums");
    p.x3_big = !bf16_gemm && y.wide && gemm_x3_on && gemm_bf16_big(R, Cn);
    p.ns = fam == BwdFamily::Overlapped ? dw_slabs_per_dir
           : p.dw_bias_out && gemm_tile256(p.dw_rows, Cn) ? pick_split_mc(p.dw_rows, Cn, ndir)
           : p.dw_from_bf16 && gemm_tile256(R, Cn) ? pick_split_mc(R, Cn, ndir)
           : (bf16_gemm || p.x3_big) && gemm_bf16_big(R, Cn) ? pick_split(R, Cn, ndir, GB2_BT) : pick_split(R, Cn, ndir);
    return p;
  }
  bool backward_weight_gradient(int l, const BwdPlan& p, const ReduceTarget& rt) {
    Layer& y = L[l];
    hipStream_t s = stream();
    const int M = ndir * 4 * y.no, R = 1 + y.ni + y.no, Cn = 4 * y.no;
    const bool product = p.family != BwdFamily::Overlapped, stacked = L.size() > 1;
    DevBuf<float>& pbuf = layer_partial(y);
    const char* const bracket = product ? "gemm_gates_dw" : stacked ? nullptr : "reduce_scatter";
    if (bracket) timing.begin(bracket, s);
    bool dx_done = false;
    if (product) {
      pbuf.reserve((size_t)ndir * p.ns * R * Cn);
      const GemmOperand src = gemm_batched(gemm_mc(y.S.p, y.lds, N), (long long)N * y.lds, ndir);
      const GemmOperand dlt = gemm_batched(gemm_mc(y.D.p, M, N, 0), 4LL * y.no, 1);
      const StorePartial store{pbuf.p, R, Cn};
      if (p.dw_from_bf16) dx_done = backward_dw_bf16(l, p, pbuf.p);
      else if (bf16_gemm) gemm_bf16<GEMM_MC, GEMM_MC>(s, src, dlt, store, R, Cn, (int)N, p.ns, ndir);
      else if (p.x3_big) gemm_x3_big<GEMM_MC, GEMM_MC>(s, src, dlt, store, R, Cn, (int)N, p.ns, ndir);
      else gemm_f32<GEMM_MC, GEMM_MC, StorePartial, GEMM_BK_DW>(s, src, dlt, store, R, Cn, (int)N, p.ns, ndir);
    }
    const ReduceDesc gates{pbuf.p, y.moff, 0LL, p.ns, ndir, R, Cn, y.no};
    const ReduceDesc extra = l == (int)L.size() - 1 ? sm_red : ReduceDesc{};
    if (stacked) pending_red.push_back(PendingReduce{gates, extra});
    else reduce_layer(gates, extra, true, rt);
    if (bracket) timing.end(s);
    check_launch();
    return dx_done;
  }
  bool backward_dw_bf16(int l, const BwdPlan& p, float* slabs) {
    Layer& y = L[l];
    hipStream_t s = stream();
    const int M = ndir * 4 * y.no, R = 1 + y.ni + y.no, Cn = 4 * y.no, ldsb = y.ni + y.no + 8;
    g_path_count[PC_DW_FROM_BF16]++;
    const GemmOperand16B src{y.Sbf.p, ldsb, (long long)N * ndir * ldsb, (long long)N * ldsb}, dlt{y.Dbf.p, M, (long long)N * M, 4LL * y.no};
    const GemmOperand16B a2 = y.sbf_x_external ? GemmOperand16B{L[l - 1].Hbf.p, y.ni, (long long)N * y.ni, 0} : GemmOperand16B{nullptr, 0, 0, 0};
    const int a2_rows = y.sbf_x_external ? y.ni : 0;
    bool dx_done = false;
    if (!p.dw_bias_out) gemm_b16mc(s, src, dlt, StorePartialRot{slabs, R, Cn}, R, Cn, (int)N, p.ns, ndir, a2, a2_rows);
    else {
      const StorePartialShift store{slabs, R, Cn};
      float* const dxp = l > 0 ? L[l - 1].dH.p : nullptr;
      dx_done = dxp && y.bwd_exact && y.Wtb.p &&
                gemm_dw_dx(s, src, dlt, store, p.dw_rows, Cn, (int)N, p.ns, ndir, a2, a2_rows, GemmOperand16{y.Dbf.p, M, (long long)N * M},
                           GemmOperand16{y.Wtb.p, M, (long long)y.ni * M}, StorePlain{dxp, y.ni}, (int)N, y.ni, M);
      if (!dx_done) gemm_b16mc(s, src, dlt, store, p.dw_rows, Cn, (int)N, p.ns, ndir, a2, a2_rows);
      CLSTM_LAUNCH(k_bias_rows, dim3((unsigned)(((size_t)ndir * Cn + 63) / 64)), dim3(64), 0, s, (const float*)y.dbias.p, slabs, bs, ndir, p.ns, R, Cn);
      g_path_count[PC_DW_BIAS_OUT]++;
      if (dx_done) { g_path_count[PC_DX_FROM_BF16]++; g_path_count[PC_DW_DX_ONE_LAUNCH]++; }
    }
    if (y.sbf_x_external) g_path_count[PC_DW_X_EXTERNAL]++;
    return dx_done;
  }
  void backward_input_deltas(int l, const BwdPlan& p) {
    Layer& y = L[l];
    hipStream_t s = stream();
    const int M = ndir * 4 * y.no;
    if (l == 0 && want_dx0) dX0.reserve((size_t)N * y.ni);
    float* const dx = l > 0 ? L[l - 1].dH.p : want_dx0 ? dX0.p : nullptr;
    if (!dx) return;
    timing.begin("gemm_gates_dx", s);
    if (bf16_gemm && bf16_rec && p.bwd_persistent && y.bwd_exact && y.Wtb.p && y.Dbf.p) {
      g_path_count[PC_DX_FROM_BF16]++;
      gemm_b16kk(s, GemmOperand16{y.Dbf.p, M, (long long)N * M}, GemmOperand16{y.Wtb.p, M, (long long)y.ni * M}, StorePlain{dx, y.ni}, (int)N, y.ni, M);
    } else if (ensure_delta_f32(l), bf16_gemm)
      gemm_bf16<GEMM_KC, GEMM_KC>(s, gemm_kc(y.D.p, M, N, 32), gemm_kc(y.Wt, M, y.ni, y.wt_slack), StorePlain{dx, y.ni}, (int)N, y.ni, M);
    else if (y.wide && gemm_x3_on && gemm_bf16_big((int)N, y.ni))
      gemm_x3_big<GEMM_KC, GEMM_KC>(s, gemm_kc(y.D.p, M, N, 32), gemm_kc(y.Wt, M, y.ni, y.wt_slack), StorePlain{dx, y.ni}, (int)N, y.ni, M);
    else
      gemm_f32<GEMM_KC, GEMM_KC>(s, gemm_kc(y.D.p, M, N), gemm_kc(y.Wt, M, y.ni, 0), StorePlain{dx, y.ni}, (int)N, y.ni, M);
    timing.end(s);
    check_launch();
  }
  struct PendingReduce { ReduceDesc gates, extra; };
  std::vector<PendingReduce> pending_red;
  void launch_deferred_reduce(DeferredReduce& deferred, const IngestTail* tail) {
    if (!deferred.armed) return;
    deferred.armed = false;
    const int nb = nblocks(deferred.work);
    timing.begin("reduce_scatter", deferred.q);
    if (tail) {
      IngestTail t = *tail;
      t.nb_main = nb;
      const int ntrail = (t.lo_src ? 1 : 0) + (t.aux_src ? (t.aux_n + 255) / 256 : 0);
      CLSTM_LAUNCH(k_reduce_scatter_ingest, dim3(nb + t.nbi + ntrail), dim3(256), 0, deferred.q, deferred.gates, deferred.extra, deferred.gdst, (int*)nullptr, 0, deferred.uf, t);
      g_path_count[PC_INGEST_TAIL]++;
    } else {
      CLSTM_LAUNCH(k_reduce_scatter, dim3(nb), dim3(256), 0, deferred.q, deferred.gates, deferred.extra, deferred.gdst, (int*)nullptr, 0, deferred.uf);
    }
    timing.end(deferred.q);
    check_launch();
  }
  struct NextBatch {
    bool valid = false;
    const float* x = nullptr;
    std::vector<int> T, labels, L;
    static size_t nlabels(const Minibatch& m) {
      size_t nl = 0;
      for (int b = 0; b < m.bs; b++) nl += (size_t)m.L[b];
      return nl;
    }
    bool matches(const Minibatch& m) const {
      if (!valid || x != m.x || (int)T.size() != m.bs) return false;
      if (memcmp(T.data(), m.T, (size_t)m.bs * sizeof(int)) || memcmp(L.data(), m.L, (size_t)m.bs * sizeof(int))) return false;
      const size_t nl = nlabels(m);
      return nl == labels.size() && (nl == 0 || !memcmp(labels.data(), m.labels, nl * sizeof(int)));
    }
    void remember(const Minibatch& m) {
      x = m.x; T.assign(m.T, m.T + m.bs); L.assign(m.L, m.L + m.bs);
      labels.assign(m.labels, m.labels + nlabels(m));
      valid = true;
    }
  } next;
  DevBuf<float>& layer_partial(Layer& y) { return L.size() > 1 ? y.partial : partial; }
  void reduce_layer(const ReduceDesc& gates, const ReduceDesc& extra, bool last, const ReduceTarget& rt) {
    hipStream_t q = stream();
    const size_t work = (size_t)gates.nbatch * gates.R * gates.Cn + (size_t)extra.R * extra.Cn * extra.nbatch;
    UpdateFuse uf{};
    uf.nanflag = nanflag(); uf.step_no = step_no();
    PassLeft& left = rt.left;
    if (rt.plan.fuse) {
      uf = UpdateFuse{v, d, lr, mom, gclip, (const int*)dev_err_words(), last ? left.ticket.word : nullptr, left.ticket.id, nanflag(), step_no(), PackDst{}};
      if (last) { left.ticket.word = nullptr; left.update_applied = true; }
      left.packs_follow_update = false;
      if (L.size() == 1 && !L[0].wide && !packed_dirty && pack_inverse(L[0])) {
        Layer& y = L[0];
        const size_t nr = (size_t)ndir * 4 * 4 * y.nk4 * y.nthreads;
        uf.pk = PackDst{y.pack_inv.p, PACK_KD, y.Wt, y.bias, y.Rf, y.Rb, y.pd, pack_fused_desc(y), (unsigned)((size_t)(1 + y.ni) * ndir * 4 * y.no), (unsigned)nr};
        left.packs_follow_update = true;
        g_path_count[PC_PACKS_FOLLOW_UPDATE]++;
      }
    }
    if (rt.plan.defer_last && last && rt.plan.fuse) {
      left.deferred = DeferredReduce{true, gates, extra, rt.gdst, uf, work, q};
      return;
    }
    CLSTM_LAUNCH(k_reduce_scatter, dim3(nblocks(work)), dim3(256), 0, q, gates, extra, rt.gdst, (int*)nullptr, 0, uf);
    if (rt.plan.peer && last) left.peer_pending = true;
  }

  long long nbackward = 0;
  int step_no() const { return (int)std::min<long long>(nbackward, 2147483647LL); }
  bool training = true;
  int* fwd_nanflag() const { return training && !in_predict ? nanflag() : nullptr; }
  static int* nanflag() {
    static const bool on = !(getenv("CLSTM_NANCHECK") && atoi(getenv("CLSTM_NANCHECK")) == 0);
    return on ? dev_err_words() + 3 : nullptr;
  }
  bool fuse_eligible() const { return !comm || comm->nranks == 1; }
  StepPlan step_plan(bool next_given, const HostTicket* ticket) {
    StepPlan p;
    p.fuse = fuse_eligible();
    p.peer = comm && comm->nranks > 1 && comm->peer_ready((size_t)nparams, stream());
    p.defer_last = next_given && p.fuse;
    if (ticket) p.ticket = *ticket;
    return p;
  }
  void update(PassLeft& left) {
    hipStream_t s = stream();
    RoctxRange range_("clstm:update");
    params_epoch++;
    if (left.update_applied) {
      packed_dirty = !left.packs_follow_update;
      return;
    }
    HostTicket& tk = left.ticket;
    if (left.peer_pending) {
      RoctxRange range2_("clstm:allreduce+update");
      const int sq = ++comm->peer.seq;
      const bool two = peer_use_two_phase((size_t)nparams, comm->nranks);
      timing.begin("allreduce_grads", s);
      peer_exchange_begin(*comm, sq, two, (size_t)nparams, s);
      timing.end(s);
      timing.begin("sgd_update", s);
      peer_exchange_finish(*comm, sq, two, v, d, g, (size_t)nparams, lr, mom, gclip, (const int*)dev_err_words(), tk.word, tk.id, nanflag(),
                           step_no(), s);
      tk.word = nullptr;
      timing.end(s);
      check_launch();
      g_path_count[PC_PEER_EXCHANGE]++;
      if (two) g_path_count[PC_PEER_TWO_PHASE]++;
      packed_dirty = true;
      maybe_replica_check(s);
      return;
    }
    if (comm && comm->nranks > 1) {
      RoctxRange range2_("clstm:allreduce");
      timing.begin("allreduce_grads", s);
      comm->allreduce(g, nparams, s);
      timing.end(s);
    }
    timing.begin("sgd_update", s);
    CLSTM_LAUNCH(k_update, dim3(nblocks(nparams)), dim3(256), 0, s, v, d, (const float*)g, (size_t)nparams, lr, mom, gclip, (const int*)dev_err_words(), tk.word, tk.id,
                 nanflag(), step_no());
    tk.word = nullptr;
    timing.end(s);
    check_launch();
    packed_dirty = true;
    if (comm && comm->nranks > 1) maybe_replica_check(s);
  }
  long long nupdates_dp = 0;
  static int replica_every() {
    static const int n = getenv("CLSTM_REPLICA_CHECK_EVERY") ? atoi(getenv("CLSTM_REPLICA_CHECK_EVERY")) : 256;
    return n;
  }
  void maybe_replica_check(hipStream_t s) {
    nupdates_dp++;
    const int every = replica_every();
    if (every > 0 && nupdates_dp % every == 0) replica_check(s);
  }
  void replica_check(hipStream_t s) {
    if (!comm || comm->nranks < 2) return;
    RoctxRange range_("clstm:replica_check");
    comm->chk.reserve(8);
    comm->chk_acc.reserve(2);
    CLSTM_LAUNCH(k_param_checksum, dim3(std::min<unsigned>(nblocks(nparams), 1024u)), dim3(256), 0, s, (const float*)v, (size_t)nparams, comm->chk_acc.p);
    CLSTM_LAUNCH(k_checksum_pieces, dim3(1), dim3(64), 0, s, comm->chk_acc.p, comm->chk.p);
    comm->allreduce(comm->chk.p + 4, 4, s, true);
    CLSTM_LAUNCH(k_replica_verify, dim3(1), dim3(64), 0, s, (const float*)comm->chk.p, comm->nranks, dev_err_words() + 7, step_no());
    check_launch();
    g_path_count[PC_REPLICA_CHECK]++;
  }
};
```

clstm_amd/csrc/ops.h:

```cpp
#pragma once
#include "devintrin.h"

namespace clstm {

enum { LIN = 0, SIG = 1, TANH = 2, RELU = 3, LOGMAG = 4 };

DEVFN float nonlin_fwd(float x, int nl) {
  switch (nl) {
    case SIG: return sigmoid_dev(x);
    case TANH: return tanh_dev(x);
    case RELU: return x > 0.0f ? x : 0.0f;
    case LOGMAG: return logf(fabsf(x) + 1.0f) * ((x < 0.0f ? 1.0f : 0.0f) * -2.0f + 1.0f);
    default: return x;
  }
}
DEVFN float nonlin_deriv(float y, int nl) {
  switch (nl) {
    case SIG: return y * (-y + 1.0f);
    case TANH: return -y * y + 1.0f;
    case RELU: return y > 0.0f ? 1.0f : 0.0f;
    case LOGMAG: return expf(-fabsf(y));
    default: return 1.0f;
  }
}
// ... 431 lines not shown
  CLSTM_GRID_STRIDE(e, nf + nb) {
    float x = 0.0f;
    if (e < nf) {
      const int k = e % kp;
      const size_t q = e / kp;
      const int row = q % rows_f, dir = q / rows_f;
      const int cell = row >> 2, slot = row & 3;
      if (cell < p.no && k < p.no) x = v[p.p_off[dir][slot] + cell + (size_t)p.no * (1 + p.ni + k)];
      Rbf[e] = (unsigned short)(bf16_pack2(x, 0.0f) & 0xFFFFu);
    } else {
      const size_t e2 = e - nf;
      const int col = e2 % kpb;
      const size_t q = e2 / kpb;
      const int k = q % rows_b, dir = q / rows_b;
      const int j = col >> 2, slot = col & 3;
      if (j < p.no && k < p.no) x = v[p.p_off[dir][slot] + j + (size_t)p.no * (1 + p.ni + k)];
      Rbb[e2] = (unsigned short)(bf16_pack2(x, 0.0f) & 0xFFFFu);
    }
  }
}

__global__ void k_pack_wide_split(const float* v, unsigned short* Rb2, PackDesc p, int rows_b, int kpb, long long plane) {
  const size_t nb = (size_t)p.ndir * rows_b * kpb;
  CLSTM_GRID_STRIDE(e, nb) {
    float x = 0.0f;
    const int col = e % kpb;
    const size_t q = e / kpb;
    const int k = q % rows_b, dir = q / rows_b;
    const int j = col >> 2, slot = col & 3;
    if (j < p.no && k < p.no) x = v[p.p_off[dir][slot] + j + (size_t)p.no * (1 + p.ni + k)];
    const unsigned hi = bf16_pack2(x, 0.0f) & 0xFFFFu;
    Rb2[e] = (unsigned short)hi;
    Rb2[e + plane] = (unsigned short)(bf16_pack2(x - __builtin_bit_cast(float, hi << 16), 0.0f) & 0xFFFFu);
  }
}

__global__ __launch_bounds__(256) void k_pack_wide_tiles(const float* v, PackDesc p, float* Wt, float* bias, unsigned short* Wtb,
                                                        unsigned short* WtbT, unsigned short* Rbf, unsigned short* Rbb, int kf, int kb,
                                                        int rows_f, int rows_b) {
  __shared__ __attribute__((aligned(16))) float tile[32 * 132];
  const int no = p.no, ni = p.ni, M = p.ndir * 4 * no;
  const int nct = no >> 5, nkx = ni >> 5, nk = nkx + (no >> 5);
  int b = blockIdx.x;
  const int ct = b % nct; b /= nct;
  const int kt = b % nk, dir = b / nk;
  const bool isx = kt < nkx;
  const int k0 = (isx ? kt : kt - nkx) << 5, c0 = ct << 5;
  const int tid = threadIdx.x;
  {
    const int cell = tid & 31, q = tid >> 5;
    float x[16];
#pragma unroll
    for (int i = 0; i < 16; i++) {
      const int g = i & 3, cc = q + 8 * (i >> 2);
      x[i] = v[p.p_off[dir][g] + (c0 + cell) + (size_t)no * (1 + (isx ? 0 : ni) + k0 + cc)];
    }
#pragma unroll
    for (int i = 0; i < 16; i++) tile[(q + 8 * (i >> 2)) * 132 + cell * 4 + (i & 3)] = x[i];
  }
  if (isx && kt == 0 && tid < 128) bias[dir * 4 * no + 4 * c0 + tid] = v[p.p_off[dir][tid & 3] + c0 + (tid >> 2)];
  __syncthreads();
  {
    const int cc = tid >> 3, ch = tid & 7;
    const int k = k0 + cc;
    float x[16];
#pragma unroll
    for (int j = 0; j < 4; j++) {
      const f32x4 t = *reinterpret_cast<const f32x4*>(&tile[cc * 132 + ch * 16 + j * 4]);
      x[4 * j] = t[0]; x[4 * j + 1] = t[1]; x[4 * j + 2] = t[2]; x[4 * j + 3] = t[3];
    }
    float lo8[8], hi8[8];
#pragma unroll
    for (int j = 0; j < 8; j++) { lo8[j] = x[j]; hi8[j] = x[8 + j]; }
    const int col0 = 4 * (c0 + 4 * ch);
    if (isx) {
      float* wt = Wt + (size_t)k * M + dir * 4 * no + col0;
#pragma unroll
      for (int j = 0; j < 4; j++) *reinterpret_cast<f32x4*>(wt + 4 * j) = f32x4{x[4 * j], x[4 * j + 1], x[4 * j + 2], x[4 * j + 3]};
      unsigned short* wb = Wtb + (size_t)k * M + dir * 4 * no + col0;
      *reinterpret_cast<u16x8*>(wb) = bf16_pack8(lo8);
      *reinterpret_cast<u16x8*>(wb + 8) = bf16_pack8(hi8);
    } else {
      unsigned short* rb = Rbb + ((size_t)dir * rows_b + k) * kb + col0;
      *reinterpret_cast<u16x8*>(rb) = bf16_pack8(lo8);
      *reinterpret_cast<u16x8*>(rb + 8) = bf16_pack8(hi8);
    }
  }
  {
    const int r = tid >> 1, hf = tid & 1;
    float lo8[8], hi8[8];
#pragma unroll
    for (int j = 0; j < 8; j++) { lo8[j] = tile[(hf * 16 + j) * 132 + r]; hi8[j] = tile[(hf * 16 + 8 + j) * 132 + r]; }
    const size_t row = (size_t)4 * c0 + r;
    unsigned short* dst = isx ? WtbT + ((size_t)dir * 4 * no + row) * ni + k0 + hf * 16
                              : Rbf + ((size_t)dir * rows_f + row) * kf + k0 + hf * 16;
    *reinterpret_cast<u16x8*>(dst) = bf16_pack8(lo8);
    *reinterpret_cast<u16x8*>(dst + 8) = bf16_pack8(hi8);
  }
}

__global__ void k_build_source(float* S, const float* x, size_t N, int ni, int ldx, int lds, int ndir, long long sdir) {
  CLSTM_GRID_STRIDE(e, N * (size_t)(1 + ni)) {
    const size_t n = e / (1 + ni);
    const int j = e % (1 + ni);
    const float v = j == 0 ? 1.0f : x[n * ldx + (j - 1)];
    for (int d = 0; d < ndir; d++) S[(size_t)d * sdir + n * lds + j] = v;
  }
}
__global__ void k_h_from_state(float* H, const float* G, const float* C, size_t N, int no, int ndir, int ldh, int hofs) {
  CLSTM_GRID_STRIDE(e, N * (size_t)ndir * no) {
    const size_t n = e / ((size_t)ndir * no);
    const int r = e % ((size_t)ndir * no);
    H[n * ldh + hofs + r] = tanh_fast(C[e]) * G[e * 4 + 2];
  }
}
__global__ void k_source_h(float* S, const float* H, const int* line_off, int bs, size_t N, int no, int ndir, int ldh, int hofs,
                           int lds, int sofs, long long sdir) {
  CLSTM_GRID_STRIDE(e, N * (size_t)ndir * no) {
    const size_t n = e / ((size_t)ndir * no);
    const int r = e % ((size_t)ndir * no), dir = r / no, cell = r % no;
    int lo = 0, hi = bs;
    while (hi - lo > 1) { const int mid = (lo + hi) >> 1; if ((size_t)line_off[mid] <= n) lo = mid; else hi = mid; }
    const long long off = line_off[lo], T = line_off[lo + 1] - off, t = (long long)n - off;
    const long long prev = dir == 0 ? t - 1 : t + 1;
    S[(size_t)dir * sdir + n * lds + sofs + cell] = (prev >= 0 && prev < T) ? H[(off + prev) * ldh + hofs + r] : 0.0f;
  }
}
struct ReduceDesc {
  const float* partial;
  const long long* moff;
  long long base;
  int nsplit, nbatch, R, Cn, rs;
};
struct PackDst {
  const int* inv; int kd;
  float *Wt, *bias, *Rf, *Rb;
  PackDesc p; PackFused pf;
  unsigned nwx, nr;
};
DEVFN void pack_dst_store(const PackDst& k, unsigned e, float x) {
  if (e < k.nwx) pack_wx_store(e, x, k.Wt, k.bias, k.p);
  else if (e < k.nwx + k.nr) k.Rf[e - k.nwx] = x;
  else if (e < k.nwx + 2 * k.nr) k.Rb[e - k.nwx - k.nr] = x;
  else pack_fused_store(e - k.nwx - 2 * k.nr, x, k.pf, k.p);
}
struct UpdateFuse {
  float* v; float* d;
  float lr, mom, clip;
  const int* err;
  int* step_word; int step_id;
  int* nanflag; int step_no;
  PackDst pk;
};
DEVFN void reduce_scatter_one(const ReduceDesc& d, size_t e, float* g, const UpdateFuse& u, const bool apply) {
  const size_t RC = (size_t)d.R * d.Cn;
  const int b = e / RC;
  const int rc = e - b * RC;
  const int r = rc / d.Cn, c = rc % d.Cn;
  const float* p = d.partial + (size_t)b * d.nsplit * RC + rc;
  float s[8] = {0.0f, 0.0f, 0.0f, 0.0f, 0.0f, 0.0f, 0.0f, 0.0f};
  int z = 0;
  for (; z + 8 <= d.nsplit; z += 8) {
    float x[8];
#pragma unroll
    for (int u = 0; u < 8; u++) x[u] = p[(size_t)(z + u) * RC];
#pragma unroll
    for (int u = 0; u < 8; u++) s[u] += x[u];
  }
  {
    float x[8];
#pragma unroll
    for (int u = 0; u < 8; u++) x[u] = z + u < d.nsplit ? p[(size_t)(z + u) * RC] : 0.0f;
#pragma unroll
    for (int u = 0; u < 8; u++) s[u] += x[u];
  }
  const long long o = (d.moff ? d.moff[(size_t)b * d.Cn + c] : d.base + c) + (long long)d.rs * r;
  const float gv = ((s[0] + s[1]) + (s[2] + s[3])) + ((s[4] + s[5]) + (s[6] + s[7]));
  g[o] = gv;
  bool fin = true;
  if (u.nanflag && !f32_finite(gv)) { raise_nonfinite(u.nanflag, u.step_no); fin = false; }
  if (apply && fin) {
    float di = u.d[o] + gv;
    if (u.clip < 1e6f) di = fmaxf(-u.clip, fminf(u.clip, di));
    const float nv = u.v[o] + di * u.lr;
    u.v[o] = nv;
    u.d[o] = di * u.mom;
    if (u.pk.inv) {
      const int* ip = u.pk.inv + (size_t)o * u.pk.kd;
      for (int k = 0; k < u.pk.kd; k++) {
        const int e = ip[k];
        if (e < 0) break;
        pack_dst_store(u.pk, (unsigned)e, nv);
      }
    }
  }
}
__global__ void k_bias_rows(const float* dbias, float* partial, int bs, int ndir, int nsplit, int R, int Cn) {
  CLSTM_GRID_STRIDE(e, (size_t)ndir * Cn) {
    const int dir = e / Cn, c = e % Cn;
    const float* p = dbias + (size_t)dir * Cn + c;
    const size_t ls = (size_t)ndir * Cn;
    float s[8] = {0.0f, 0.0f, 0.0f, 0.0f, 0.0f, 0.0f, 0.0f, 0.0f};
    for (int b = 0; b < bs; b += 8) {
      float x[8];
#pragma unroll
      for (int u = 0; u < 8; u++) x[u] = b + u < bs ? p[(size_t)(b + u) * ls] : 0.0f;
#pragma unroll
      for (int u = 0; u < 8; u++) s[u] += x[u];
    }
    const float t = ((s[0] + s[1]) + (s[2] + s[3])) + ((s[4] + s[5]) + (s[6] + s[7]));
    for (int z = 0; z < nsplit; z++) partial[(((size_t)dir * nsplit + z) * R) * Cn + c] = z == 0 ? t : 0.0f;
  }
}
DEVFN void reduce_scatter_blocks(const ReduceDesc& d0, const ReduceDesc& d1, float* g, int* zero, const int zero_n, const UpdateFuse& u, const unsigned nb) {
  if (zero && blockIdx.x == 0 && (int)threadIdx.x < zero_n) zero[threadIdx.x] = 0;
  if (u.step_word && blockIdx.x == 0 && threadIdx.x == 0) store_i32_wt(u.step_word, u.step_id);
  const bool apply = u.v && !dev_err_set(u.err);
  const size_t n0 = (size_t)d0.R * d0.Cn * d0.nbatch, n1 = (size_t)d1.R * d1.Cn * d1.nbatch;
  for (size_t e = (size_t)blockIdx.x * blockDim.x + threadIdx.x; e < n0 + n1; e += (size_t)nb * blockDim.x) {
    if (e < n0) reduce_scatter_one(d0, e, g, u, apply);
    else reduce_scatter_one(d1, e - n0, g, u, apply);
  }
}
__global__ void k_reduce_scatter(ReduceDesc d0, ReduceDesc d1, float* g, int* zero, int zero_n, UpdateFuse u) {
  reduce_scatter_blocks(d0, d1, g, zero, zero_n, u, gridDim.x);
}
__global__ void k_debug_lane_ops(float* out) {
  const int lane = threadIdx.x & 63;
  const float x = (float)lane;
  out[0 * 64 + lane] = quad_xor1(x);
  out[1 * 64 + lane] = quad_xor2(x);
  out[2 * 64 + lane] = quad_bcast<0>(x);
  out[3 * 64 + lane] = quad_bcast<1>(x);
  out[4 * 64 + lane] = quad_bcast<2>(x);
  out[5 * 64 + lane] = quad_bcast<3>(x);
  out[6 * 64 + lane] = row_ror<1>(x);
  out[7 * 64 + lane] = row_ror<4>(x);
  out[8 * 64 + lane] = row_ror<8>(x);
  out[9 * 64 + lane] = row_half_mirror(x);
  out[10 * 64 + lane] = wave_shr1(x);
}
__global__ void k_ingest(const float* x, float* X, float* S, size_t N, int ni, int lds, int ndir, long long sdir) {
  CLSTM_GRID_STRIDE(e, N * (size_t)(1 + ni)) {
    const size_t n = e / (1 + ni);
    const int j = e % (1 + ni);
    float v = 1.0f;
    if (j > 0) {
      v = x[n * ni + (j - 1)];
      X[n * ni + (j - 1)] = v;
    }
    for (int d = 0; d < ndir; d++) S[(size_t)d * sdir + n * lds + j] = v;
  }
}
__global__ void k_bf16_to_f32(const unsigned short* src, float* dst, size_t n) {
  CLSTM_GRID_STRIDE(e, n) dst[e] = __builtin_bit_cast(float, (unsigned)src[e] << 16);
}
__global__ void k_to_bf16(const float* src, unsigned short* dst, size_t n) {
  CLSTM_GRID_STRIDE(e, n) dst[e] = (unsigned short)(bf16_pack2(src[e], 0.0f) & 0xFFFFu);
}

__global__ void k_source_one_bf16(unsigned short* Sbf, size_t N, int one_col, int ldsb, int ndir, long long sbdir) {
  CLSTM_GRID_STRIDE(n, N) {
    u16x8 v;
#pragma unroll
    for (int i = 0; i < 8; i++) v[i] = (unsigned short)(i == 0 ? 0x3F80 : 0);
    for (int d = 0; d < ndir; d++) *reinterpret_cast<u16x8*>(&Sbf[(size_t)d * sbdir + n * ldsb + one_col]) = v;
  }
}
__global__ void k_source_x_bf16(unsigned short* Sbf, const float* xf, const unsigned short* xb, int ldx, size_t N, int ni, int one_col,
                                int ldsb, int ndir, long long sbdir) {
  const int cpr = (ni >> 3) + 1;
  CLSTM_GRID_STRIDE(e, N * (size_t)cpr) {
    const size_t n = e / cpr;
    const int j = (int)(e - n * cpr);
    u16x8 v;
    int col = j * 8;
    if (j < (ni >> 3)) {
      if (xb) v = *reinterpret_cast<const u16x8*>(&xb[n * ldx + col]);
      else {
        float x[8];
#pragma unroll
        for (int i = 0; i < 8; i++) x[i] = xf[n * ldx + col + i];
        v = bf16_pack8(x);
      }
    } else {
      col = one_col;
#pragma unroll
      for (int i = 0; i < 8; i++) v[i] = (unsigned short)(i == 0 ? 0x3F80 : 0);
    }
    for (int d = 0; d < ndir; d++) *reinterpret_cast<u16x8*>(&Sbf[(size_t)d * sbdir + n * ldsb + col]) = v;
  }
}

__global__ void k_transpose_to_bf16(const float* src, unsigned short* dst, int rows, int cols) {
  CLSTM_GRID_STRIDE(e, (size_t)rows * cols) {
    const int c = (int)(e / rows), k = (int)(e % rows);
    dst[e] = (unsigned short)(bf16_pack2(src[(size_t)k * cols + c], 0.0f) & 0xFFFFu);
  }
}

DEVFN void ingest_rows(const float* x, float* X, float* S, const size_t N, const int ni, const int lds, const int ndir, const long long sdir,
                       const unsigned blk, const unsigned nbi) {
  if ((ni & 3) == 0 && (lds & 3) == 0 && ((size_t)x & 15) == 0) {
    const size_t nch = (size_t)ni / 4 + 1;
    for (size_t e = (size_t)blk * blockDim.x + threadIdx.x; e < N * nch; e += (size_t)nbi * blockDim.x) {
      const size_t n = e / nch;
      const int c = (int)(e - n * nch);
      const float prev = c == 0 ? 1.0f : x[n * ni + 4 * c - 1];
      if (4 * c < ni) {
        const f32x4 xv = *reinterpret_cast<const f32x4*>(x + n * ni + 4 * c);
        *reinterpret_cast<f32x4*>(X + n * ni + 4 * c) = xv;
        const f32x4 sv = f32x4{prev, xv[0], xv[1], xv[2]};
        for (int d = 0; d < ndir; d++) *reinterpret_cast<f32x4*>(S + (size_t)d * sdir + n * lds + 4 * c) = sv;
      } else {
        for (int d = 0; d < ndir; d++) S[(size_t)d * sdir + n * lds + 4 * c] = prev;
      }
    }
  } else {
    for (size_t e = (size_t)blk * blockDim.x + threadIdx.x; e < N * (size_t)(1 + ni); e += (size_t)nbi * blockDim.x) {
      const size_t n = e / (1 + ni);
      const int j = e % (1 + ni);
      float val = 1.0f;
      if (j > 0) {
        val = x[n * ni + (j - 1)];
        X[n * ni + (j - 1)] = val;
      }
      for (int d = 0; d < ndir; d++) S[(size_t)d * sdir + n * lds + j] = val;
    }
  }
}
DEVFN void ingest_small(int blk, const int* lo_src, int* lo_dst, const int lo_n, const int* aux_src, int* aux_dst, const int aux_n) {
  if (lo_src) {
    if (blk == 0) {
      for (int i = threadIdx.x; i < lo_n; i += blockDim.x) lo_dst[i] = lo_src[i];
      return;
    }
    blk--;
  }
  const int i = blk * (int)blockDim.x + (int)threadIdx.x;
  if (i < aux_n) aux_dst[i] = aux_src[i];
}
__global__ void k_ingest_pack(const float* x, float* X, float* S, size_t N, int ni, int lds, int ndir, long long sdir,
                              int nbi, int nbp, const float* v, float* Wt, float* bias, float* Rf, float* Rb, PackDesc p, PackFused pf,
                              const int* lo_src, int* lo_dst, int lo_n, const int* aux_src, int* aux_dst, int aux_n, const int* tab) {
  if ((int)blockIdx.x >= nbi + nbp) { ingest_small((int)blockIdx.x - (nbi + nbp), lo_src, lo_dst, lo_n, aux_src, aux_dst, aux_n); return; }
  if ((int)blockIdx.x < nbi) {
    ingest_rows(x, X, S, N, ni, lds, ndir, sdir, blockIdx.x, (unsigned)nbi);
  } else {
// ... 56 lines not shown
```

clstm_amd/csrc/runtime.inc:

```

static thread_local std::string g_err;
static thread_local hipStream_t g_stream = nullptr;

struct Error : std::runtime_error {
  using std::runtime_error::runtime_error;
};
#define HIPCHECK(expr)                                                                       \
  do {                                                                                       \
    hipError_t e_ = (expr);                                                                  \
    if (e_ != hipSuccess)                                                                    \
      throw Error(std::string(#expr) + " failed: " + hipGetErrorString(e_) + " (" + __FILE__ + \
                  ":" + std::to_string(__LINE__) + ")");                                     \
  } while (0)
#define REQUIRE(cond, msg)                    \
  do {                                        \
    if (!(cond)) throw Error(std::string(msg)); \
  } while (0)
#define ABI_BEGIN try {
#define ABI_END                         \
  return 0;                             \
  }                                     \
  catch (const std::exception& e) {     \
    g_err = e.what();                   \
    return 1;                           \
  }                                     \
  catch (...) {                         \
    g_err = "unknown error";            \
    return 1;                           \
  }

static inline int nblocks(size_t n, int bs = 256) {
  size_t b = (n + bs - 1) / bs;
  if (b < 1) b = 1;
  if (b > 4096) b = 4096;
  return (int)b;
}
static void check_launch() { HIPCHECK(hipGetLastError()); }

static void zero_fill(void* p, size_t bytes) {
  HIPCHECK(hipMemsetAsync(p, 0, bytes, g_stream));
  HIPCHECK(hipStreamSynchronize(g_stream));
}
static thread_local size_t* g_acct = nullptr;
struct AcctScope {
  size_t* prev;
  explicit AcctScope(size_t* c) : prev(g_acct) { g_acct = c; }
  ~AcctScope() { g_acct = prev; }
};
template <class T>
struct DevBuf {
  T* p = nullptr;
  size_t cap = 0;
  size_t* acct = g_acct;
  void reserve(size_t n) {
    if (n <= cap) return;
    if (p) HIPCHECK(hipFree(p));
    p = nullptr;
    if (acct) *acct -= cap * sizeof(T);
    cap = 0;
    size_t want = n + n / 4 + 64;
    HIPCHECK(hipMalloc((void**)&p, want * sizeof(T)));
    zero_fill(p, want * sizeof(T));
    cap = want;
    if (acct) *acct += cap * sizeof(T);
  }
  void release() {
    if (p) (void)hipFree(p);
    p = nullptr;
    if (acct) *acct -= cap * sizeof(T);
    cap = 0;
  }
};

struct PinnedRing {
  static const int SLOTS = 32, GROUP = 8;
  void* h[SLOTS] = {};
  size_t cap[SLOTS] = {};
  hipEvent_t ev[SLOTS / GROUP] = {};
  bool busy[SLOTS / GROUP] = {};
  int cur = SLOTS - 1;
  void* acquire(size_t bytes) {
    cur = (cur + 1) % SLOTS;
    const int g = cur / GROUP;
    if (cur % GROUP == 0 && busy[g]) { HIPCHECK(hipEventSynchronize(ev[g])); busy[g] = false; }
    if (cap[cur] < bytes) {
      if (h[cur]) (void)hipHostFree(h[cur]);
      cap[cur] = bytes * 2 + 256;
      HIPCHECK(hipHostMalloc(&h[cur], cap[cur]));
    }
    return h[cur];
  }
  void commit(hipStream_t s) {
    if (cur % GROUP != GROUP - 1) return;
    const int g = cur / GROUP;
    if (!ev[g]) HIPCHECK(hipEventCreateWithFlags(&ev[g], hipEventDisableTiming));
    HIPCHECK(hipEventRecord(ev[g], s));
    busy[g] = true;
  }
  ~PinnedRing() {
    for (int i = 0; i < SLOTS / GROUP; i++)
      if (ev[i]) (void)hipEventDestroy(ev[i]);
    for (int i = 0; i < SLOTS; i++)
      if (h[i]) (void)hipHostFree(h[i]);
  }
};
template <class T>
struct PinnedBuf {
  T* p = nullptr;
  size_t cap = 0;
  void reserve(size_t n) {
    if (n <= cap) return;
    if (p) HIPCHECK(hipHostFree(p));
    p = nullptr; cap = 0;
    HIPCHECK(hipHostMalloc((void**)&p, (n + n / 4 + 64) * sizeof(T)));
    cap = n + n / 4 + 64;
  }
  PinnedBuf() = default;
  PinnedBuf(const PinnedBuf&) = delete;
  ~PinnedBuf() { if (p) (void)hipHostFree(p); }
};

struct StoreBias {
  float* out; long long ld; const float* bias;
  DEVMFN void operator()(int r, int c, float v, int) const { out[(long long)r * ld + c] = v + bias[c]; }
  DEVMFN bool vec4() const { return (ld & 3) == 0 && (((size_t)out | (size_t)bias) & 15) == 0; }
  DEVMFN void row4(int r, int c, f32x4 v, int) const {
    const f32x4 b = *reinterpret_cast<const f32x4*>(bias + c);
    f32x4 o;
    o[0] = v[0] + b[0]; o[1] = v[1] + b[1]; o[2] = v[2] + b[2]; o[3] = v[3] + b[3];
    *reinterpret_cast<f32x4*>(out + (long long)r * ld + c) = o;
  }
};
enum PathCounter {
  PC_FWD_PERSISTENT = 0, PC_BWD_PERSISTENT = 1, PC_WX_FROM_BF16 = 2, PC_DX_FROM_BF16 = 3, PC_DW_FROM_BF16 = 4, PC_FWD_FUSED = 5,
  PC_FWD_FUSED_WX = 6, PC_PEER_EXCHANGE = 7, PC_DW_X_EXTERNAL = 8, PC_BWD_C32 = 9, PC_PACKS_FOLLOW_UPDATE = 10, PC_BWD_X3 = 11,
  PC_REPLICA_CHECK = 12, PC_DW_BIAS_OUT = 13, PC_DW_DX_ONE_LAUNCH = 14, PC_MFMA_NOSAVE = 15, PC_MFMA_FWD = 16, PC_MFMA_BWD = 17,
  PC_MFMA_BWD_DW = 18, PC_INGEST_TAIL = 19, PC_INGEST_TAIL_USED = 20, PC_MFMA_ROUTED = 21 ,
  PC_LINE_NOSAVE = 22, PC_FUSED_NOSAVE = 23, PC_PEER_TWO_PHASE = 24, PC_NORMALIZED = 25, PC_XD_PROLOGUE = 26, PC_XD_PRODUCERS = 27, PC_SCORE = 28, PC_BEAM = 29, PC_COUNT
};
static long long g_path_count[PC_COUNT];
struct StorePlain {
  float* out; long long ld;
  DEVMFN void operator()(int r, int c, float v, int) const { out[(long long)r * ld + c] = v; }
  DEVMFN bool vec4() const { return (ld & 3) == 0 && ((size_t)out & 15) == 0; }
  DEVMFN void row4(int r, int c, f32x4 v, int) const { *reinterpret_cast<f32x4*>(out + (long long)r * ld + c) = v; }
};
struct StorePartial {
  float* out; int R, Cn;
  DEVMFN void operator()(int r, int c, float v, int z) const { out[((long long)z * R + r) * Cn + c] = v; }
  DEVMFN bool vec4() const { return (Cn & 3) == 0 && ((size_t)out & 15) == 0; }
  DEVMFN void row4(int r, int c, f32x4 v, int z) const {
    *reinterpret_cast<f32x4*>(out + ((long long)z * R + r) * Cn + c) = v;
  }
};
struct StorePartialShift {
  float* out; int R, Cn;
  DEVMFN void operator()(int r, int c, float v, int z) const { out[((long long)z * R + r + 1) * Cn + c] = v; }
  DEVMFN bool vec4() const { return (Cn & 3) == 0 && ((size_t)out & 15) == 0; }
  DEVMFN void row4(int r, int c, f32x4 v, int z) const { *reinterpret_cast<f32x4*>(out + ((long long)z * R + r + 1) * Cn + c) = v; }
};
struct StorePartialRot {
  float* out; int R, Cn;
  DEVMFN void operator()(int r, int c, float v, int z) const { out[((long long)z * R + (r + 1 == R ? 0 : r + 1)) * Cn + c] = v; }
  DEVMFN bool vec4() const { return (Cn & 3) == 0 && ((size_t)out & 15) == 0; }
  DEVMFN void row4(int r, int c, f32x4 v, int z) const {
    *reinterpret_cast<f32x4*>(out + ((long long)z * R + (r + 1 == R ? 0 : r + 1)) * Cn + c) = v;
  }
};
#ifndef GEMM_BK_DW
#define GEMM_BK_DW 16
#endif
#define NARROW_CLASSES(X) X(1, 4, 0, 0, 0) X(2, 8, 0, 0, 0) X(4, 16, 0, 1, 1) X(7, 25, 1, 1, 1) X(7, 28, 1, 1, 0) X(8, 32, 1, 1, 1)
#define MFMA_GEOMS(X) X(64, 1, 1) X(100, 1, 1) X(128, 0, 0)
struct NarrowClass { int nk4, ku, waves; bool fused, dw, routed; };
static NarrowClass narrow_class(int no) {
  const int k4 = (no + 3) / 4, waves = (no + 15) / 16;
#define ROW_(N, K, F, D, R) if (4 * N >= k4 && (K == 4 * N || K == k4)) return NarrowClass{N, K, waves, F != 0, D != 0, R != 0};
  NARROW_CLASSES(ROW_)
#undef ROW_
  return NarrowClass{0, 0, 1, false, false, false};
}
struct MfmaGeomCaps { int no; bool nosave, bwd; };
static const MfmaGeomCaps* mfma_geom(int no) {
#define ROW_(NO, NOSAVE, BWD) {NO, NOSAVE != 0, BWD != 0},
  static const MfmaGeomCaps table[] = {MFMA_GEOMS(ROW_)};
#undef ROW_
  for (const auto& g : table)
    if (g.no == no) return &g;
  return nullptr;
}
[[noreturn]] static void no_instantiation() { throw Error("internal: the plan names a recurrence kernel that is not instantiated"); }
template <int N, int K> struct NarrowNK { static constexpr int NK4 = N, KU = K; };
enum NarrowCap { NCAP_LINE, NCAP_FUSED, NCAP_DW, NCAP_ROUTED };
template <int CAP, class F>
static void narrow_dispatch(int nk4, int ku, F&& f) {
#define CASE_(N, K, FUSED, DW, ROUTED) \
  if constexpr (CAP == NCAP_LINE || (CAP == NCAP_FUSED && FUSED) || (CAP == NCAP_DW && DW) || (CAP == NCAP_ROUTED && ROUTED)) \
    if (nk4 == N && ku == K) { f(NarrowNK<N, K>{}); check_launch(); return; }
  NARROW_CLASSES(CASE_)
#undef CASE_
  no_instantiation();
}
enum MfmaCap { MCAP_FWD, MCAP_NOSAVE, MCAP_BWD };
template <int CAP, class F>
static void mfma_dispatch(int no, F&& f) {
#define CASE_(NO, NOSAVE, BWD) \
  if constexpr (CAP == MCAP_FWD || (CAP == MCAP_NOSAVE && NOSAVE) || (CAP == MCAP_BWD && BWD)) \
    if (no == NO) { f(std::integral_constant<int, NO>{}); check_launch(); return; }
  MFMA_GEOMS(CASE_)
#undef CASE_
  no_instantiation();
}
template <int NK4, int KU, bool SAVE = true>
static void launch_fwd(const LstmSeqArgs& a, int bs, int nthreads, hipStream_t s) {
  const size_t smem = (2 * 4 * (size_t)lstm_qstride(NK4) + 4) * sizeof(float);
  CLSTM_LAUNCH((lstm_fwd_kernel<NK4, KU, SAVE>), dim3(bs, a.ndir), dim3(nthreads), smem, s, a);
}
template <int NK4, int KU>
static void launch_bwd(const LstmSeqArgs& a, int bs, int nthreads, hipStream_t s) {
  const size_t smem = (2 * 16 * (size_t)lstm_qstride(NK4) + 4) * sizeof(float);
  CLSTM_LAUNCH((lstm_bwd_kernel<NK4, KU>), dim3(bs, a.ndir), dim3(nthreads), smem, s, a);
}
template <int NK4, int KU, bool SAVE = true>
static void launch_fwd_fused(const FwdFusedKernelArgs& k, unsigned nblk, int nthreads, hipStream_t s) {
  const size_t smem = (2 * 4 * (size_t)lstm_qstride(NK4) + 4) * sizeof(float);
#ifdef CLSTM_HIP_EMU
  CLSTM_LAUNCH_COOP((lstm_fwd_fused_kernel<NK4, KU, SAVE>), dim3(nblk), dim3(nthreads), smem, s, k);
#else
  CLSTM_LAUNCH((lstm_fwd_fused_kernel<NK4, KU, SAVE>), dim3(nblk), dim3(nthreads), smem, s, k);
#endif
}
static void launch_lstm_fwd_fused(int nk4, int ku, const FwdFusedKernelArgs& k, unsigned nblk, int nthreads, hipStream_t s, bool save = true) {
  narrow_dispatch<NCAP_FUSED>(nk4, ku, [&](auto c) {
    constexpr int N = decltype(c)::NK4, K = decltype(c)::KU;
    if (save) launch_fwd_fused<N, K>(k, nblk, nthreads, s); else launch_fwd_fused<N, K, false>(k, nblk, nthreads, s);
  });
}
static void launch_lstm(bool fwd, int nk4, int ku, const LstmSeqArgs& a, int bs, int nthreads, hipStream_t s, bool save = true) {
  narrow_dispatch<NCAP_LINE>(nk4, ku, [&](auto c) {
    constexpr int N = decltype(c)::NK4, K = decltype(c)::KU;
    if (!fwd) launch_bwd<N, K>(a, bs, nthreads, s); else if (save) launch_fwd<N, K>(a, bs, nthreads, s); else launch_fwd<N, K, false>(a, bs, nthreads, s);
  });
}
static void launch_lstm_bwd_xd(int nk4, int ku, const LstmSeqArgs& a, const XdArgs& x, int terms, int bs, int nthreads, hipStream_t s) {
  narrow_dispatch<NCAP_LINE>(nk4, ku, [&](auto c) {
    constexpr int N = decltype(c)::NK4, K = decltype(c)::KU;
    const size_t smem = (2 * 16 * (size_t)lstm_qstride(N) + 4) * sizeof(float);
    if (terms >= 3) CLSTM_LAUNCH((lstm_bwd_xd_kernel<N, K, 3>), dim3(bs, a.ndir), dim3(nthreads), smem, s, a, x);
    else CLSTM_LAUNCH((lstm_bwd_xd_kernel<N, K, 2>), dim3(bs, a.ndir), dim3(nthreads), smem, s, a, x);
  });
}
static void launch_lstm_bwd_dw(int nk4, int ku, const LstmSeqArgs& a, const GemmDwArgs& g, int terms, int nrec, unsigned ngemm, int nthreads, hipStream_t s) {
  narrow_dispatch<NCAP_DW>(nk4, ku, [&](auto c) {
    constexpr int N = decltype(c)::NK4, K = decltype(c)::KU;
    const size_t smem = (2 * 16 * (size_t)lstm_qstride(N) + 4) * sizeof(float);
    if (terms >= 3) CLSTM_LAUNCH((lstm_bwd_dw_kernel<N, K, 3>), dim3(nrec + ngemm), dim3(nthreads), smem, s, a, g, nrec);
    else if (terms) CLSTM_LAUNCH((lstm_bwd_dw_kernel<N, K, 2>), dim3(nrec + ngemm), dim3(nthreads), smem, s, a, g, nrec);
    else CLSTM_LAUNCH((lstm_bwd_dw_kernel<N, K, 0>), dim3(nrec + ngemm), dim3(nthreads), smem, s, a, g, nrec);
  });
}
static void launch_gemm_dw(const GemmDwArgs& g, int terms, unsigned nblk, hipStream_t s) {
  if (terms >= 3) CLSTM_LAUNCH(gemm_dw_kernel<3>, dim3(nblk), dim3(256), 0, s, g);
  else if (terms) CLSTM_LAUNCH(gemm_dw_kernel<2>, dim3(nblk), dim3(256), 0, s, g);
  else CLSTM_LAUNCH(gemm_dw_kernel<0>, dim3(nblk), dim3(256), 0, s, g);
  check_launch();
}

static int device_cu_count() {
#ifndef CLSTM_HIP_EMU
  static int n = [] {
    int dev = 0, v = 0;
    if (hipGetDevice(&dev) != hipSuccess) return 0;
    if (hipDeviceGetAttribute(&v, hipDeviceAttributeMultiprocessorCount, dev) != hipSuccess) return 0;
    return v;
  }();
  return n;
#else
  static const int n = getenv("CLSTM_EMU_CUS") ? atoi(getenv("CLSTM_EMU_CUS")) : 16;
  return n;
#endif
}
template <class K>
static void coop_set_smem(K kernel, size_t smem) {
#ifndef CLSTM_HIP_EMU
  HIPCHECK(hipFuncSetAttribute((const void*)kernel, hipFuncAttributeMaxDynamicSharedMemorySize, (int)smem));
#endif
}
struct StepGraphCache {
  bool unsupported = false;
#ifndef CLSTM_HIP_EMU
  struct Entry { std::vector<char> key; int kind; int tmax; hipGraphExec_t exec; };
  std::vector<Entry> entries;
  hipGraphExec_t find(int kind, const std::vector<char>& key, int tmax) {
    for (auto& e : entries)
      if (e.kind == kind && e.tmax == tmax && e.key == key) return e.exec;
    return nullptr;
  }
  void put(int kind, const std::vector<char>& key, int tmax, hipGraphExec_t exec) {
    if (entries.size() >= 16) { (void)hipGraphExecDestroy(entries.front().exec); entries.erase(entries.begin()); }
    entries.push_back(Entry{key, kind, tmax, exec});
  }
  ~StepGraphCache() { for (auto& e : entries) (void)hipGraphExecDestroy(e.exec); }
#endif
};
template <class A>
static std::vector<char> graph_key(A a) {
  a.step = 0;
  std::vector<char> k(sizeof(A));
  memcpy(k.data(), &a, sizeof(A));
  return k;
}
template <class A, class F>
static void launch_steps(StepGraphCache& cache, int kind, const A& a, int tmax, hipStream_t s, F&& body) {
#ifndef CLSTM_HIP_EMU
  if (tmax >= 8) {
    const std::vector<char> key = graph_key(a);
    hipGraphExec_t exec = cache.find(kind, key, tmax);
    if (!exec && !cache.unsupported) {
      hipGraph_t graph = nullptr;
      if (hipStreamBeginCapture(s, hipStreamCaptureModeThreadLocal) != hipSuccess) {
        (void)hipGetLastError();
        cache.unsupported = true;
      } else {
        body();
        HIPCHECK(hipStreamEndCapture(s, &graph));
        HIPCHECK(hipGraphInstantiate(&exec, graph, nullptr, nullptr, 0));
        HIPCHECK(hipGraphDestroy(graph));
        cache.put(kind, key, tmax, exec);
      }
    }
    if (exec) {
      HIPCHECK(hipGraphLaunch(exec, s));
      return;
    }
  }
#endif
  body();
}
static int* g_dev_err = nullptr;
static int* dev_err_words() {
  if (!g_dev_err) {
    HIPCHECK(hipMalloc((void**)&g_dev_err, 16 * sizeof(int)));
    zero_fill(g_dev_err, 16 * sizeof(int));
  }
  return g_dev_err;
}
static bool g_xcd_failed = false;
struct XcdOutcome {
  static const int SLOTS = 16;
  volatile int* pinned = nullptr;
  bool pending[SLOTS] = {};
  int next = 0, verified = 0;
  void check_slot(int i) {
    if (!pending[i]) return;
    if (pinned[i] == -1) {
      const auto t0 = std::chrono::steady_clock::now();
      while (pinned[i] == -1 && std::chrono::steady_clock::now() - t0 < std::chrono::seconds(20)) sched_yield();
      if (pinned[i] == -1) { HIPCHECK(hipDeviceSynchronize()); }
    }
    pending[i] = false;
    const int e = pinned[i];
    if (e > 0 && g_dev_err) (void)hipMemset(g_dev_err, 0, sizeof(int));
    if (e == 1) g_xcd_failed = true;
    if (e > 0)
      throw Error(e == 1 ? "persistent recurrence: the workgroups of a later launch were not all resident / not spread evenly over the XCDs (another process or stream on the device?); "
                           "the minibatches enqueued since then were NOT applied -- every later update was skipped; in a multi-layer net the layers above the failing one may "
                           "have taken their update of that one minibatch -- and the library has switched to the per-step launches (CLSTM_XCD_REC=0) for the rest of the process"
                         : "persistent recurrence: a group barrier timed out in the middle of the sequence; the minibatches enqueued since then were NOT applied (layers above the "
                           "failing one may have taken their update of that one minibatch) -- set CLSTM_XCD_REC=0");
  }
  void check_all() { for (int i = 0; i < SLOTS; i++) check_slot(i); }
  int* prepare() {
#ifdef CLSTM_HIP_EMU
    return nullptr;
#else
    if (verified < 4) return nullptr;
    if (!pinned) { int* p = nullptr; HIPCHECK(hipHostMalloc((void**)&p, SLOTS * sizeof(int))); pinned = p; }
    const int i = next;
    next = (next + 1) % SLOTS;
    check_slot(i);
    pinned[i] = -1;
    pending[i] = true;
    return (int*)(pinned + i);
#endif
  }
  bool after_launch(const int* last_err_d, hipStream_t s) {
#ifdef CLSTM_HIP_EMU
    if (*last_err_d != 0 && g_dev_err) g_dev_err[0] = 0;
    if (*last_err_d == 2) throw Error("persistent recurrence: group barrier timed out");
    return *last_err_d == 0;
#else
    if (verified < 4) {
      int flag = 0;
      HIPCHECK(hipMemcpyAsync(&flag, last_err_d, sizeof(int), hipMemcpyDeviceToHost, s));
      HIPCHECK(hipStreamSynchronize(s));
      if (flag == 0) { verified++; return true; }
      if (g_dev_err) (void)hipMemset(g_dev_err, 0, sizeof(int));
      if (flag != 1) throw Error("persistent recurrence: a group barrier timed out in the middle of the sequence; set CLSTM_XCD_REC=0");
      return false;
    }
    return true;
#endif
  }
};
static XcdOutcome g_xcd_outcome;
static void check_device_errors() {
  g_xcd_outcome.check_all();
  if (!g_dev_err) return;
  int w[8] = {0, 0, 0, 0, 0, 0, 0, 0};
  HIPCHECK(hipMemcpy(w, g_dev_err, sizeof(w), hipMemcpyDeviceToHost));
  if ((w[0] | w[1] | w[2] | w[3] | w[6] | w[7]) == 0) return;
// ... 343 lines not shown
```

clstm_amd/csrc/step.inc:

```

static void net_ingest(Net& n, CtcWorkspace& ctc, const float* x, const CtcMetaCopy* aux = nullptr) {
  REQUIRE(n.N > 0, "set_batch first");
  n.ensure_training_buffers();
  RoctxRange range_("clstm:ingest");
  Layer& y = n.L[0];
  bool aux_done = false;
  const bool with_pack = n.packed_dirty && n.L.size() == 1 && !y.wide;
  if (with_pack || n.lo_pending || (aux && aux->nwords > 0)) {
    const int M = n.ndir * 4 * y.no, KQP = 4 * y.nk4;
    const size_t nr = (size_t)n.ndir * 4 * KQP * y.nthreads;
    const int nbi = n.ingest_blocks(x), nbp = with_pack ? nblocks((size_t)(1 + y.ni) * M + 2 * nr) : 0;
    const bool lo = n.lo_pending, ax = aux && aux->nwords > 0;
    CLSTM_LAUNCH(k_ingest_pack, dim3(nbi + nbp + (lo ? 1 : 0) + (ax ? (aux->nwords + 255) / 256 : 0)), dim3(256), 0, g_stream, x, n.X.p, y.S.p, (size_t)n.N, y.ni, y.lds,
                 n.ndir, (long long)n.N * y.lds, nbi, nbp, (const float*)n.v, y.Wt, y.bias, y.Rf, y.Rb, y.pd, n.pack_fused_desc(y),
                 lo ? n.lo_stage : nullptr, n.line_off.p, 2 * n.bs + 1, ax ? aux->src : nullptr, ax ? aux->dst : nullptr, ax ? aux->nwords : 0,
                 with_pack ? (const int*)n.pack_table(y) : (const int*)nullptr);
    if (lo) { n.ring.commit(g_stream); n.lo_pending = false; }
    if (ax) { ctc.ring.commit(g_stream); aux_done = true; }
    if (with_pack) n.packed_dirty = false;
  } else {
    CLSTM_LAUNCH(k_ingest, dim3(nblocks((size_t)n.N * (1 + y.ni))), dim3(256), 0, g_stream, x, n.X.p, y.S.p, (size_t)n.N, y.ni,
                 y.lds, n.ndir, (long long)n.N * y.lds);
  }
  check_launch();
  if (aux && aux->nwords > 0 && !aux_done) {
    HIPCHECK(hipMemcpyAsync(aux->dst, aux->src, (size_t)aux->nwords * sizeof(int), hipMemcpyHostToDevice, g_stream));
    ctc.ring.commit(g_stream);
  }
  n.src0_ready = true;
}
static IngestTail ingest_tail(const Net& n, const float* x, const CtcMetaCopy& meta) {
  const Layer& y = n.L[0];
  IngestTail t{};
  t.x = x; t.X = n.X.p; t.S = y.S.p; t.N = (unsigned long long)n.N; t.ni = y.ni; t.lds = y.lds; t.ndir = n.ndir; t.sdir = (long long)n.N * y.lds;
  t.nbi = n.ingest_blocks(x);
  t.lo_src = n.lo_pending ? n.lo_stage : nullptr; t.lo_dst = n.line_off.p; t.lo_n = 2 * n.bs + 1;
  t.aux_src = meta.nwords > 0 ? meta.src : nullptr; t.aux_dst = meta.dst; t.aux_n = meta.nwords;
  return t;
}
static void net_ctc(Net& n, CtcWorkspace& ctc, const Minibatch& m, float* aligned_h, CtcMetaCopy* defer = nullptr, bool launch = true) {
  REQUIRE(n.N > 0, "set_batch first");
  std::vector<int> soff, states;
  expand_transcripts(m.labels, m.L, n.bs, states, soff);
  float* al = nullptr;
  if (aligned_h) { n.aligned.reserve((size_t)n.N * n.desc.nclasses); al = n.aligned.p; }
  RoctxRange range_(launch ? "clstm:ctc" : "clstm:ctc_prepare");
  if (launch) n.timing.begin("ctc_align", g_stream);
  run_ctc(ctc, n.Z.p, n.Dz.p, al, n.desc.nclasses, n.line_off_h.data(), states.data(), soff.data(), n.bs, g_stream, defer, launch);
  if (launch) n.timing.end(g_stream);
  if (aligned_h && launch) copy_d2h(aligned_h, al, (size_t)n.N * n.desc.nclasses);
}
static void net_ctc_launch(Net& n, CtcWorkspace& ctc) {
  RoctxRange range_("clstm:ctc");
  n.timing.begin("ctc_align", g_stream);
  launch_ctc_align(ctc, g_stream);
  n.timing.end(g_stream);
}

static void train_step(Net& n, CtcWorkspace& ctc, const Minibatch& cur, const Minibatch& next, const HostTicket* ticket) {
  if (!ticket && n.next.matches(cur) && n.src0_ready && !n.lo_pending) {
    n.next.valid = false;
    g_path_count[PC_INGEST_TAIL_USED]++;
  } else {
    n.set_batch(cur.T, cur.bs);
    CtcMetaCopy meta;
    net_ctc(n, ctc, cur, nullptr, &meta, false);
    net_ingest(n, ctc, cur.x, &meta);
  }
  n.forward();
  net_ctc_launch(n, ctc);
  PassLeft left = n.backward(n.step_plan(next.given(), ticket));
  if (left.deferred.armed) {
    bool tail = !(n.L.size() == 1 && !n.L[0].wide && !left.packs_follow_update);
    if (tail) {
      try {
        n.set_batch(next.T, next.bs);
        CtcMetaCopy meta;
        net_ctc(n, ctc, next, nullptr, &meta, false);
        const IngestTail t = ingest_tail(n, next.x, meta);
        n.launch_deferred_reduce(left.deferred, &t);
        if (t.lo_src) { n.ring.commit(g_stream); n.lo_pending = false; }
        if (t.aux_src) ctc.ring.commit(g_stream);
        n.src0_ready = true;
        n.next.remember(next);
      } catch (...) {
        n.next.valid = false;
        tail = false;
      }
    }
    if (!tail) n.launch_deferred_reduce(left.deferred, nullptr);
  }
  n.update(left);
  if (ticket) {
    REQUIRE(left.ticket.word == nullptr, "internal: no kernel of the step took the step word");
    n.hf.commit();
  }
}
```

Baseline: 232,800.

## Fold deferred gradient reduce and next-batch ingest into the fused backward-dw launch

Adds a 'reduce role' to the fused LSTM backward weight-gradient kernel. Extra trailing blocks wait on slab-completion counters, sum the split partials (early slabs first, the tail slabs later), apply the fused momentum update, and ingest the next batch. This removes the separate deferred reduce/ingest launch and overlaps the reduction with the tail of the gradient GEMM. In exchange it adds spin-waiting blocks, write-through stores and system-scope error checks, plus more complex progress bookkeeping with watchdog fallbacks.

```diff
diff --git a/clstm_amd/csrc/dbgopt.h b/clstm_amd/csrc/dbgopt.h
--- a/clstm_amd/csrc/dbgopt.h
+++ b/clstm_amd/csrc/dbgopt.h
@@ -18,6 +18,7 @@
     {"gemm_x3", 1},
     {"split_terms", 3},
     {"xd_prologue", 2},
+    {"reduce_role", 1},
     {"fwd_mfma", 1},
     {"bwd_mfma", 1},
     {"bwd_mfma_fused", 1},
diff --git a/clstm_amd/csrc/devintrin.h b/clstm_amd/csrc/devintrin.h
--- a/clstm_amd/csrc/devintrin.h
+++ b/clstm_amd/csrc/devintrin.h
@@ -295,6 +295,9 @@
 #endif
 
 DEVFN bool dev_err_set(const int* err) { return err && (err[0] | err[1] | err[2] | err[3] | err[6] | err[7]) != 0; }
+DEVFN bool dev_err_set_sys(const int* err) {
+  return err && (load_i32_wt(err) | load_i32_wt(err + 1) | load_i32_wt(err + 2) | load_i32_wt(err + 3) | load_i32_wt(err + 6) | load_i32_wt(err + 7)) != 0;
+}
 DEVFN bool f32_finite(float x) { return (__builtin_bit_cast(unsigned, x) & 0x7f800000u) != 0x7f800000u; }
 DEVFN void raise_nonfinite(int* nanflag, int step_no) { if (*nanflag == 0) *nanflag = step_no; }
 
diff --git a/clstm_amd/csrc/gemm_dw.h b/clstm_amd/csrc/gemm_dw.h
--- a/clstm_amd/csrc/gemm_dw.h
+++ b/clstm_amd/csrc/gemm_dw.h
@@ -9,7 +9,8 @@
   int need_it;
   int dir;
   int out_z;
-  int pad[3];
+  int tail;
+  int pad[2];
 };
 
 struct XdArgs {
@@ -47,6 +48,7 @@
   int x3;
   int terms;
   XdArgs xd;
+  int* slab_done;
 };
 
 constexpr int DW_PF = 3;
@@ -92,6 +94,7 @@
       break;
     }
   }
+  if (a.slab_done && lane == 0) atomic_add_i32(a.slab_done + PROG_STRIDE, 1);
 }
 
 DEVFN void gemm_dw_wait(const GemmDwArgs& a, const int dir, const int need_it) {
@@ -116,6 +119,20 @@
   __syncthreads();
 }
 
+DEVFN void dw_store_wt(float* out, const int pR, const int pCn, const int r, const int c, const f32x4 v, const bool v4) {
+  const BufF32 ob = make_buf(out, (size_t)pR * pCn * 4);
+  const unsigned off = ((unsigned)r * (unsigned)pCn + (unsigned)c) * 4u;
+  if (v4 && c + 3 < pCn) buf_store4_wt(ob, off, v);
+  else
+    for (int e = 0; e < 4; e++)
+      if (c + e < pCn) buf_store_wt(ob, off + 4u * e, v[e]);
+}
+DEVFN void dw_slab_publish(const GemmDwArgs& a, const DwSlab& sl) {
+  if (!a.slab_done) return;
+  drain_vmem();
+  __syncthreads();
+  if (threadIdx.x == 0) atomic_add_i32(a.slab_done + (sl.tail ? PROG_STRIDE : 0), 1);
+}
 DEVFN void gemm_dw_item(const GemmDwArgs& a, float* smem, const unsigned si, const unsigned tile) {
   float* As = smem;
   float* Bs = smem + GEMM_BK * GEMM_LD;
@@ -207,12 +224,14 @@
     const int r = r0 + rl, c = c0 + cl;
     const f32x4 v = *reinterpret_cast<const f32x4*>(&smem[rl * GEMM_LDO + cl]);
     if (r < a.R) {
-      if (v4 && c + 3 < a.Cn) *reinterpret_cast<f32x4*>(out + (size_t)r * a.Cn + c) = v;
+      if (a.slab_done) dw_store_wt(out, a.R, a.Cn, r, c, v, v4);
+      else if (v4 && c + 3 < a.Cn) *reinterpret_cast<f32x4*>(out + (size_t)r * a.Cn + c) = v;
       else
         for (int e = 0; e < 4; e++)
           if (c + e < a.Cn) out[(size_t)r * a.Cn + c + e] = v[e];
     }
   }
+  dw_slab_publish(a, sl);
 }
 template <int NT>
 DEVFN void gemm_dw_item_x3(const GemmDwArgs& a, float* smem, const unsigned si, const unsigned tile, const bool extra = false) {
@@ -351,12 +370,14 @@
     const int r = r0 + rl, c = c0 + cl;
     const f32x4 v = *reinterpret_cast<const f32x4*>(&smem[rl * GEMM_LDO + cl]);
     if (r < pR) {
-      if (v4 && c + 3 < pCn) *reinterpret_cast<f32x4*>(out + (size_t)r * pCn + c) = v;
+      if (a.slab_done) dw_store_wt(out, pR, pCn, r, c, v, v4);
+      else if (v4 && c + 3 < pCn) *reinterpret_cast<f32x4*>(out + (size_t)r * pCn + c) = v;
       else
         for (int e = 0; e < 4; e++)
           if (c + e < pCn) out[(size_t)r * pCn + c + e] = v[e];
     }
   }
+  dw_slab_publish(a, sl);
   if (a.trace && tid == 0 && !extra) {
     long long* tr = a.trace + ((size_t)a.trace_base + si * (a.gx * a.gy) + tile) * 4;
     tr[0] = t_start; tr[1] = t_ready; tr[2] = wall_clock(); tr[3] = sl.need_it;
diff --git a/clstm_amd/csrc/lstm_bwd_dw.h b/clstm_amd/csrc/lstm_bwd_dw.h
--- a/clstm_amd/csrc/lstm_bwd_dw.h
+++ b/clstm_amd/csrc/lstm_bwd_dw.h
@@ -2,6 +2,7 @@
 #include "gemm_dw.h"
 #include "lstm_seq.h"
 #include "lstm_xd_prologue.h"
+#include "ops.h"
 
 namespace clstm {
 
@@ -9,8 +10,91 @@
 static_assert(DW_FUSED_STAB_ENTRIES >= DW_STAB_MAX, "the items' k-tile table fits");
 static_assert(xd_smem_floats(2) <= dw_img_floats(2) && xd_smem_floats(3) <= dw_img_floats(3), "the recurrence role's x.d prologue stages in the items' carve");
 
+constexpr int DW_ROLE_E = 3;
+struct DwLastRole {
+  unsigned first;
+  int nb0, nb1, nbi;
+  ReduceDesc d0, d1;
+  int early0, early1;
+  float* g; UpdateFuse u;
+  IngestTail t;
+  const int* slab_done;
+  int early_target, all_target;
+  int* timeouts;
+  long long* trace;
+};
+DEVFN bool dw_role_wait(const int* word, const int target, int* timeouts, int* flag) {
+  if (threadIdx.x < 64) {
+    bool ok = true;
+    int polls = 0;
+    for (;;) {
+      if ((int)((unsigned)wave_uniform(load_i32_wt(word)) - (unsigned)target) >= 0) break;
+      if (++polls > (DW_WATCHDOG_POLLS << 4)) { ok = false; break; }
+      sleep_iterations(1);
+    }
+    if (threadIdx.x == 0) {
+      if (!ok) atomic_add_i32(timeouts, 1);
+      *flag = ok ? 1 : 0;
+    }
+  }
+  __syncthreads();
+  const bool ok = *flag != 0;
+  __syncthreads();
+  return ok;
+}
+DEVFN void dw_role_reduce(const DwLastRole& r, const ReduceDesc& d, const int ne, const unsigned blk, int* flag, long long* tr) {
+  const long long t0 = tr ? wall_clock() : 0;
+  const size_t RC = (size_t)d.R * d.Cn, n = RC * d.nbatch;
+  const unsigned RC4 = (unsigned)RC * 4u;
+  const BufF32 pb = make_buf(d.partial, n * d.nsplit * 4);
+  bool live[DW_ROLE_E];
+  unsigned poff[DW_ROLE_E];
+  long long o[DW_ROLE_E];
+  UpdatePre pre[DW_ROLE_E];
+  float s[DW_ROLE_E][8];
+#pragma unroll
+  for (int j = 0; j < DW_ROLE_E; j++) {
+    const size_t e = ((size_t)blk * DW_ROLE_E + j) * blockDim.x + threadIdx.x;
+    live[j] = e < n;
+    const ReduceElem el = reduce_elem(d, live[j] ? e : 0);
+    o[j] = el.o;
+    poff[j] = (unsigned)(((size_t)el.b * d.nsplit * RC + el.rc) * 4);
+    pre[j] = update_prefetch(r.u, el.o);
+#pragma unroll
+    for (int u = 0; u < 8; u++) s[j][u] = 0.0f;
+  }
+  if (!dw_role_wait(r.slab_done, r.early_target, r.timeouts, flag)) return;
+#pragma unroll
+  for (int j = 0; j < DW_ROLE_E; j++)
+    slab_sum_first(s[j], [&](int z, bool in) { return buf_load_wt(pb, live[j] && in ? poff[j] + (unsigned)z * RC4 : BUF_OOB); }, ne);
+  const long long t1 = tr ? wall_clock() : 0;
+  if (!dw_role_wait(r.slab_done + PROG_STRIDE, r.all_target, r.timeouts, flag)) return;
+  const long long t2 = tr ? wall_clock() : 0;
+#pragma unroll
+  for (int j = 0; j < DW_ROLE_E; j++)
+    slab_sum_rest(s[j], [&](int z, bool in) { return buf_load_wt(pb, live[j] && in ? poff[j] + (unsigned)z * RC4 : BUF_OOB); }, ne, d.nsplit);
+  const bool apply = r.u.v && !dev_err_set_sys(r.u.err);
+#pragma unroll
+  for (int j = 0; j < DW_ROLE_E; j++)
+    if (live[j]) reduce_scatter_finish(o[j], slab_chains_combine(s[j]), r.g, r.u, apply, &pre[j]);
+  if (tr && threadIdx.x == 0) { tr[0] = t0; tr[1] = t1; tr[2] = t2; tr[3] = wall_clock(); }
+}
+DEVFN void dw_last_role(const DwLastRole& r, float* gsm, unsigned blk) {
+  int* flag = reinterpret_cast<int*>(gsm);
+  const unsigned nb0 = (unsigned)r.nb0, nb1 = (unsigned)r.nb1;
+  if (blk < nb0) { dw_role_reduce(r, r.d0, r.early0, blk, flag, r.trace ? r.trace + (size_t)blk * 4 : nullptr); return; }
+  blk -= nb0;
+  if (blk < nb1) { dw_role_reduce(r, r.d1, r.early1, blk, flag, r.trace ? r.trace + (size_t)(nb0 + blk) * 4 : nullptr); return; }
+  blk -= nb1;
+  if (!dw_role_wait(r.slab_done, r.early_target, r.timeouts, flag)) return;
+  if (!dw_role_wait(r.slab_done + PROG_STRIDE, r.all_target, r.timeouts, flag)) return;
+  const IngestTail& t = r.t;
+  if ((int)blk < r.nbi) { ingest_rows(t.x, t.X, t.S, (size_t)t.N, t.ni, t.lds, t.ndir, t.sdir, blk, (unsigned)r.nbi); return; }
+  ingest_small((int)blk - r.nbi, t.lo_src, t.lo_dst, t.lo_n, t.aux_src, t.aux_dst, t.aux_n);
+}
+
 template <int NK4, int KU, int NT>
-__global__ __launch_bounds__(64 * NK4) CLSTM_TWO_WAVES_PER_SIMD void lstm_bwd_dw_kernel(LstmSeqArgs a, GemmDwArgs g, int nrec) {
+__global__ __launch_bounds__(64 * NK4) CLSTM_TWO_WAVES_PER_SIMD void lstm_bwd_dw_kernel(LstmSeqArgs a, GemmDwArgs g, int nrec, DwLastRole role) {
   __shared__ __attribute__((aligned(16))) float gsm[dw_img_floats(NT) + 2 * DW_FUSED_STAB_ENTRIES];
   if ((int)blockIdx.x < nrec) {
 #ifndef CLSTM_HIP_EMU
@@ -42,6 +126,7 @@
         if (blk > (unsigned)nrec) blk -= (unsigned)nrec;
       }
     }
+    if (role.first && blk >= role.first) { dw_last_role(role, gsm, blk - role.first); return; }
     if (threadIdx.x >= 256) return;
     gemm_dw_body<NT>(g, gsm, blk);
   }
diff --git a/clstm_amd/csrc/net.inc b/clstm_amd/csrc/net.inc
--- a/clstm_amd/csrc/net.inc
+++ b/clstm_amd/csrc/net.inc
@@ -73,9 +73,20 @@
   bool fuse = false;
   bool peer = false;
   bool defer_last = false;
+  bool next_fits = false;
   HostTicket ticket;
 };
-struct DeferredReduce { bool armed = false; ReduceDesc gates, extra; float* gdst = nullptr; UpdateFuse uf; size_t work = 0; hipStream_t q = nullptr; };
+struct DeferredReduce { bool armed = false; ReduceDesc gates, extra; float* gdst = nullptr; UpdateFuse uf; size_t work = 0; hipStream_t q = nullptr; bool role = false; };
+struct RoleLaunch {
+  bool armed = false;
+  int nk4 = 0, ku = 0, terms = 0, nrec = 0, nthreads = 0;
+  unsigned nblk = 0;
+  LstmSeqArgs a; GemmDwArgs g; DwLastRole role;
+  unsigned n_early = 0, n_all = 0;
+  unsigned n_done = 0;
+  size_t trace_rows = 0;
+  hipStream_t s = nullptr;
+};
 struct PassLeft {
   bool update_applied = false;
   bool packs_follow_update = false;
@@ -132,8 +143,12 @@
   DevBuf<int> dwx_tab;
   long long dwx_N = -1;
   int dwx_nslabs = 0, dwx_entries = 0;
-  int dw_nslabs = 0, dw_slabs_per_dir = 0, dw_ntiles_max = 0;
+  int dw_nslabs = 0, dw_slabs_per_dir = 0, dw_ntiles_max = 0, dw_early_per_dir = 0;
+  bool role_pass = false;
+  RoleLaunch role_launch;
+  unsigned role_early_total = 0, role_all_total = 0;
   int prog_base = 1024;
+  int dw_prev_tmax = 0;
   long long dw_launches = 0;
   Comm* comm = nullptr;
   struct HostFeed {
@@ -947,6 +962,7 @@
     std::vector<std::vector<int>> tab(ndir);
     struct Sl { int tb, nt, need, dir, chunk, part; };
     std::vector<std::vector<Sl>> sl(ndir);
+    dw_early_per_dir = 0;
     for (int dir = 0; dir < ndir; dir++) {
       int cs = 0;
       for (size_t c = 0; c < cb.size(); c++) {
@@ -967,6 +983,7 @@
           REQUIRE(a1 - a0 <= DW_STAB_MAX, "internal: weight-gradient slab longer than its LDS table");
           sl[dir].push_back(Sl{a0, a1 - a0, ce, dir, (int)c, p});
         }
+        if (dir == 0 && c + DW_TAIL_CHUNKS < cb.size()) dw_early_per_dir = (int)sl[0].size();
         cs = ce;
       }
     }
@@ -978,7 +995,7 @@
     for (int i = 0; i < dw_slabs_per_dir; i++)
       for (int dir = 0; dir < ndir; dir++) {
         const Sl& x = sl[dir][i];
-        slabs.push_back(DwSlab{x.tb, x.nt, x.need, dir, dir * dw_slabs_per_dir + i, {0, 0, 0}});
+        slabs.push_back(DwSlab{x.tb, x.nt, x.need, dir, dir * dw_slabs_per_dir + i, i >= dw_early_per_dir ? 1 : 0, {0, 0}});
       }
     dw_nslabs = (int)slabs.size();
     const size_t nk = (size_t)ndir * dw_ntiles_max * 2, nsw = slabs.size() * sizeof(DwSlab) / sizeof(int);
@@ -1002,7 +1019,8 @@
     const int M = ndir * 4 * y.no;
     const long long prog_off = (long long)y.D.cap - 64 - PROG_WORDS;
     REQUIRE(prog_off >= (long long)N * M, "internal: progress words overlap the deltas");
-    prog_base += tmax + 64;
+    prog_base += std::max(tmax, dw_prev_tmax) + 64;
+    dw_prev_tmax = tmax;
     dw_launches++;
     const bool prog_base_wrapped = prog_base > (1 << 30);
     if (prog_base_wrapped) prog_base = 1024;
@@ -1018,7 +1036,7 @@
     g.partial = partial.p; g.R = R; g.Cn = Cn;
     g.gx = (unsigned)((Cn + GEMM_BT - 1) / GEMM_BT); g.gy = (unsigned)((R + GEMM_BT - 1) / GEMM_BT);
     g.timeouts = dev_err_words() + 1;
-    if (!dw_queue.p) dw_queue.reserve(5 * PROG_STRIDE);
+    if (!dw_queue.p) dw_queue.reserve(6 * PROG_STRIDE);
     g.ndir = ndir;
     g.minprog = dw_queue.p + PROG_STRIDE;
     g.tcap = tmax + 32;
@@ -1049,6 +1067,28 @@
     const size_t trace_rows = (size_t)bs * ndir + (size_t)((dw_nslabs + 7) / 8) * 8 * g.gx * g.gy + 8;
     if (trace_path) { dw_trace.reserve(trace_rows * 4); g.trace = dw_trace.p; g.trace_base = bs * ndir; }
     const unsigned nblk = 1u + (np.xd == 2 ? (unsigned)(bs * ndir) : 0u) + nextra + (unsigned)((dw_nslabs + 7) / 8) * 8u * g.gx * g.gy;
+    const double slab_lim = 2147483000.0;
+    if (role_pass && np.bwd == NB_BWD_DW && (double)ndir * dw_slabs_per_dir * R * Cn * 4.0 < slab_lim &&
+        (double)sm_red.nsplit * sm_red.nbatch * sm_red.R * sm_red.Cn * 4.0 < slab_lim) {
+      RoleLaunch& rl = role_launch;
+      rl = RoleLaunch{};
+      g.done = g.minprog + 2 * PROG_STRIDE;
+      rl.n_done = (unsigned)(bs * ndir);
+      g.done_target = (int)(dw_done_total + rl.n_done);
+      g.slab_done = g.minprog + 3 * PROG_STRIDE;
+      rl.n_early = (unsigned)(ndir * dw_early_per_dir) * g.gx * g.gy + nextra;
+      rl.n_all = (unsigned)(ndir * (dw_slabs_per_dir - dw_early_per_dir)) * g.gx * g.gy + 1u;
+      rl.nk4 = y.nk4; rl.ku = y.pd.ku; rl.terms = np.terms; rl.nrec = bs * ndir; rl.nthreads = y.nthreads; rl.nblk = nblk;
+      rl.a = a; rl.g = g; rl.s = s;
+      rl.role.first = 1u + nextra + (unsigned)((dw_nslabs + 7) / 8) * 8u * g.gx * g.gy;
+      rl.role.early0 = dw_early_per_dir;
+      rl.role.early1 = sm_red.nsplit;
+      rl.role.slab_done = g.slab_done; rl.role.timeouts = g.timeouts;
+      rl.trace_rows = trace_rows;
+      rl.armed = true;
+      return;
+    }
+    role_pass = false;
     timing.begin("lstm_bwd", s);
     if (np.bwd == NB_MFMA_DW) launch_mfma_bwd(y, a, s, &g, nblk);
     else if (np.bwd == NB_BWD_DW) {
@@ -1078,7 +1118,7 @@
     int* stage = (int*)ring.acquire(((size_t)2 * dwx_entries + nsw) * sizeof(int));
     for (int e = 0; e < dwx_entries; e++) { stage[2 * e] = 16 * e; stage[2 * e + 1] = (int)std::min<long long>(16, N - 16LL * e); }
     DwSlab* sl = (DwSlab*)(stage + 2 * dwx_entries);
-    for (int i = 0; i < dwx_nslabs; i++) sl[i] = DwSlab{eps * i, std::min(eps, dwx_entries - eps * i), 0, 0, i, {0, 0, 0}};
+    for (int i = 0; i < dwx_nslabs; i++) sl[i] = DwSlab{eps * i, std::min(eps, dwx_entries - eps * i), 0, 0, i, 0, {0, 0}};
     for (int i = 0; i < dwx_nslabs; i++) REQUIRE(sl[i].ntiles <= DW_STAB_MAX, "internal: weight-gradient slab longer than its LDS table");
     HIPCHECK(hipMemcpyAsync(dwx_tab.p, stage, ((size_t)2 * dwx_entries + nsw) * sizeof(int), hipMemcpyHostToDevice, s));
     ring.commit(s);
@@ -1098,6 +1138,8 @@
     hipStream_t s = stream();
     NarrowPlan np[CLSTM_MAX_LAYERS];
     for (int l = 0; l < (int)L.size(); l++) np[l] = backward_plan_narrow(l);
+    role_launch.armed = false;
+    role_pass = reduce_role_admitted(plan, np[L.size() - 1]);
     backward_softmax(np[L.size() - 1]);
     for (int l = (int)L.size() - 1; l >= 0; l--) {
       const BwdFamily fam = L[l].wide ? BwdFamily::Wide : np[l].overlapped ? BwdFamily::Overlapped : BwdFamily::Narrow;
@@ -1254,9 +1296,45 @@
   }
   struct PendingReduce { ReduceDesc gates, extra; };
   std::vector<PendingReduce> pending_red;
+  void launch_role_backward(const IngestTail* tail) {
+    RoleLaunch& rl = role_launch;
+    REQUIRE(rl.armed, "internal: no fused backward launch is described");
+    rl.armed = false;
+    DwLastRole& r = rl.role;
+    const size_t per_block = (size_t)DW_ROLE_E * rl.nthreads;
+    const size_t n0 = (size_t)r.d0.nbatch * r.d0.R * r.d0.Cn, n1 = (size_t)r.d1.nbatch * r.d1.R * r.d1.Cn;
+    r.nb0 = (int)((n0 + per_block - 1) / per_block); r.nb1 = (int)((n1 + per_block - 1) / per_block);
+    unsigned nrole = (unsigned)(r.nb0 + r.nb1);
+    r.nbi = 0;
+    if (tail) {
+      r.t = *tail;
+      r.nbi = std::min(std::max(1, (int)((size_t)tail->nbi * 256 / rl.nthreads)), std::max(1, device_cu_count()));
+      r.t.nb_main = (int)nrole; r.t.nbi = r.nbi;
+      nrole += (unsigned)r.nbi + (tail->lo_src ? 1u : 0u) + (tail->aux_src ? (unsigned)((tail->aux_n + rl.nthreads - 1) / rl.nthreads) : 0u);
+    }
+    r.early_target = (int)(role_early_total + rl.n_early);
+    r.all_target = (int)(role_all_total + rl.n_all);
+    static const char* trace_path = getenv("CLSTM_DW_TRACE");
+    const size_t trace_rows = rl.trace_rows + (size_t)(r.nb0 + r.nb1);
+    if (trace_path) {
+      dw_trace.reserve(trace_rows * 4);
+      rl.g.trace = dw_trace.p; rl.g.trace_base = rl.nrec;
+      r.trace = dw_trace.p + rl.trace_rows * 4;
+    }
+    timing.begin("lstm_bwd", rl.s);
+    launch_lstm_bwd_dw(rl.nk4, rl.ku, rl.a, rl.g, rl.terms, rl.nrec, rl.nblk + nrole, rl.nthreads, rl.s, r);
+    timing.end(rl.s);
+    dw_done_total += rl.n_done; role_early_total += rl.n_early; role_all_total += rl.n_all;
+    g_path_count[PC_REDUCE_ROLE]++;
+    if (trace_path)
+      dump_trace(trace_path, dw_trace.p, trace_rows, rl.s,
+                 "# rows 0..%d: recurrence workgroups (start, x.d prologue returned, end); then one row per (slab, tile) item: start ready done need_it; "
+                 "from row %d on: the reduce blocks of the last role (start, early sums done, last slab seen, done); 100 MHz ticks\n", rl.nrec - 1, (int)rl.trace_rows);
+  }
   void launch_deferred_reduce(DeferredReduce& deferred, const IngestTail* tail) {
     if (!deferred.armed) return;
     deferred.armed = false;
+    if (deferred.role) { launch_role_backward(tail); return; }
     const int nb = nblocks(deferred.work);
     timing.begin("reduce_scatter", deferred.q);
     if (tail) {
@@ -1311,6 +1389,17 @@
         g_path_count[PC_PACKS_FOLLOW_UPDATE]++;
       }
     }
+    if (role_launch.armed) {
+      REQUIRE(role_pass && last && rt.plan.fuse && left.packs_follow_update && PACK_KD == PACK_KD_MAX, "internal: the last role was described for a pass that cannot take it");
+      DwLastRole& r = role_launch.role;
+      r.d0 = gates; r.d1 = extra; r.g = rt.gdst; r.u = uf;
+      if (rt.plan.defer_last) {
+        left.deferred = DeferredReduce{true, gates, extra, rt.gdst, uf, work, q, true};
+        return;
+      }
+      launch_role_backward(nullptr);
+      return;
+    }
     if (rt.plan.defer_last && last && rt.plan.fuse) {
       left.deferred = DeferredReduce{true, gates, extra, rt.gdst, uf, work, q};
       return;
@@ -1328,13 +1417,32 @@
     return on ? dev_err_words() + 3 : nullptr;
   }
   bool fuse_eligible() const { return !comm || comm->nranks == 1; }
-  StepPlan step_plan(bool next_given, const HostTicket* ticket) {
+  StepPlan step_plan(const int* next_T, int next_bs, const HostTicket* ticket) {
     StepPlan p;
     p.fuse = fuse_eligible();
     p.peer = comm && comm->nranks > 1 && comm->peer_ready((size_t)nparams, stream());
-    p.defer_last = next_given && p.fuse;
+    p.defer_last = next_T != nullptr && p.fuse;
+    p.next_fits = p.defer_last && batch_fits(next_T, next_bs);
     if (ticket) p.ticket = *ticket;
     return p;
+  }
+  bool reduce_role_admitted(const StepPlan& plan, const NarrowPlan& top) {
+    return plan.fuse && !plan.ticket.word && top.bwd == NB_BWD_DW && L.size() == 1 && !L[0].wide && !want_dx0 && (!plan.defer_last || plan.next_fits) &&
+           dbg_opt("reduce_role") != 0 && !packed_dirty && pack_inverse(L[0]);
+  }
+  bool batch_fits(const int* T_h, int nb) const {
+    if (!T_h || nb <= 0 || geom_predict) return false;
+    long long n = 0;
+    for (int b = 0; b < nb; b++) { if (T_h[b] < 0) return false; n += T_h[b]; }
+    if (n <= 0 || n >= 2147483000LL || (size_t)(2 * nb + 1) > line_off.cap) return false;
+    const size_t n_ = (size_t)n;
+    if (n_ * desc.ninput > X.cap || n_ * desc.nclasses > Z.cap || n_ * desc.nclasses > Dz.cap) return false;
+    for (auto& y : L) {
+      if (n_ * ndir * 4 * y.no > y.G.cap || n_ * ndir * y.no > y.C.cap || n_ * y.ldh + 64 + (y.Wk ? PROG_WORDS : 0) > y.H.cap) return false;
+      if (n_ * ndir * 4 * y.no + (y.wide ? 0 : PROG_WORDS + 64) > y.D.cap || n_ * ndir * y.no > y.dH.cap || n_ * ndir * y.lds + 64 > y.S.cap) return false;
+      if (y.wide && bf16_rec) return false;
+    }
+    return true;
   }
   void update(PassLeft& left) {
     hipStream_t s = stream();
diff --git a/clstm_amd/csrc/ops.h b/clstm_amd/csrc/ops.h
--- a/clstm_amd/csrc/ops.h
+++ b/clstm_amd/csrc/ops.h
@@ -607,40 +607,71 @@
   int* nanflag; int step_no;
   PackDst pk;
 };
-DEVFN void reduce_scatter_one(const ReduceDesc& d, size_t e, float* g, const UpdateFuse& u, const bool apply) {
+template <class Ld>
+DEVFN void slab_chains(float (&s)[8], Ld&& ld, int z, const int zfull, const int lo, const int hi, const bool pad) {
+  for (; z + 8 <= zfull; z += 8) {
+    float x[8];
+#pragma unroll
+    for (int u = 0; u < 8; u++) x[u] = ld(z + u, true);
+#pragma unroll
+    for (int u = 0; u < 8; u++) s[u] += x[u];
+  }
+  if (pad) {
+    float x[8];
+#pragma unroll
+    for (int u = 0; u < 8; u++) x[u] = ld(z + u, z + u >= lo && z + u < hi);
+#pragma unroll
+    for (int u = 0; u < 8; u++) s[u] += x[u];
+  }
+}
+template <class Ld>
+DEVFN void slab_sum_first(float (&s)[8], Ld&& ld, const int ne) { slab_chains(s, ld, 0, ne, 0, ne, true); }
+template <class Ld>
+DEVFN void slab_sum_rest(float (&s)[8], Ld&& ld, const int ne, const int nsplit) {
+  if (ne >= nsplit) return;
+  int z = ne & ~7;
+  if (ne & 7) { slab_chains(s, ld, z, z, ne, nsplit, true); z += 8; }
+  slab_chains(s, ld, z, nsplit, 0, nsplit, true);
+}
+DEVFN float slab_chains_combine(const float (&s)[8]) { return ((s[0] + s[1]) + (s[2] + s[3])) + ((s[4] + s[5]) + (s[6] + s[7])); }
+struct ReduceElem { int b, rc; long long o; };
+DEVFN ReduceElem reduce_elem(const ReduceDesc& d, size_t e) {
   const size_t RC = (size_t)d.R * d.Cn;
   const int b = e / RC;
   const int rc = e - b * RC;
   const int r = rc / d.Cn, c = rc % d.Cn;
-  const float* p = d.partial + (size_t)b * d.nsplit * RC + rc;
-  float s[8] = {0.0f, 0.0f, 0.0f, 0.0f, 0.0f, 0.0f, 0.0f, 0.0f};
-  int z = 0;
-  for (; z + 8 <= d.nsplit; z += 8) {
-    float x[8];
-#pragma unroll
-    for (int u = 0; u < 8; u++) x[u] = p[(size_t)(z + u) * RC];
-#pragma unroll
-    for (int u = 0; u < 8; u++) s[u] += x[u];
-  }
-  {
-    float x[8];
-#pragma unroll
-    for (int u = 0; u < 8; u++) x[u] = z + u < d.nsplit ? p[(size_t)(z + u) * RC] : 0.0f;
-#pragma unroll
-    for (int u = 0; u < 8; u++) s[u] += x[u];
-  }
-  const long long o = (d.moff ? d.moff[(size_t)b * d.Cn + c] : d.base + c) + (long long)d.rs * r;
-  const float gv = ((s[0] + s[1]) + (s[2] + s[3])) + ((s[4] + s[5]) + (s[6] + s[7]));
+  return ReduceElem{b, rc, (d.moff ? d.moff[(size_t)b * d.Cn + c] : d.base + c) + (long long)d.rs * r};
+}
+constexpr int PACK_KD_MAX = 4;
+struct UpdatePre { float d, v; int inv[PACK_KD_MAX]; };
+DEVFN UpdatePre update_prefetch(const UpdateFuse& u, const long long o) {
+  UpdatePre p{0.0f, 0.0f, {-1, -1, -1, -1}};
+  if (u.v) {
+    p.d = u.d[o]; p.v = u.v[o];
+    if (u.pk.inv)
+#pragma unroll
+      for (int k = 0; k < PACK_KD_MAX; k++) p.inv[k] = k < u.pk.kd ? u.pk.inv[(size_t)o * u.pk.kd + k] : -1;
+  }
+  return p;
+}
+DEVFN void reduce_scatter_finish(const long long o, const float gv, float* g, const UpdateFuse& u, const bool apply, const UpdatePre* pre) {
   g[o] = gv;
   bool fin = true;
   if (u.nanflag && !f32_finite(gv)) { raise_nonfinite(u.nanflag, u.step_no); fin = false; }
   if (apply && fin) {
-    float di = u.d[o] + gv;
+    float di = (pre ? pre->d : u.d[o]) + gv;
     if (u.clip < 1e6f) di = fmaxf(-u.clip, fminf(u.clip, di));
-    const float nv = u.v[o] + di * u.lr;
+    const float nv = (pre ? pre->v : u.v[o]) + di * u.lr;
     u.v[o] = nv;
     u.d[o] = di * u.mom;
-    if (u.pk.inv) {
+    if (u.pk.inv && pre) {
+#pragma unroll
+      for (int k = 0; k < PACK_KD_MAX; k++) {
+        const int e = pre->inv[k];
+        if (e < 0) break;
+        pack_dst_store(u.pk, (unsigned)e, nv);
+      }
+    } else if (u.pk.inv) {
       const int* ip = u.pk.inv + (size_t)o * u.pk.kd;
       for (int k = 0; k < u.pk.kd; k++) {
         const int e = ip[k];
@@ -649,6 +680,14 @@
       }
     }
   }
+}
+DEVFN void reduce_scatter_one(const ReduceDesc& d, size_t e, float* g, const UpdateFuse& u, const bool apply) {
+  const size_t RC = (size_t)d.R * d.Cn;
+  const ReduceElem el = reduce_elem(d, e);
+  const float* p = d.partial + (size_t)el.b * d.nsplit * RC + el.rc;
+  float s[8] = {0.0f, 0.0f, 0.0f, 0.0f, 0.0f, 0.0f, 0.0f, 0.0f};
+  slab_chains(s, [&](int z, bool in) { return in ? p[(size_t)z * RC] : 0.0f; }, 0, d.nsplit, 0, d.nsplit, true);
+  reduce_scatter_finish(el.o, slab_chains_combine(s), g, u, apply, nullptr);
 }
 __global__ void k_bias_rows(const float* dbias, float* partial, int bs, int ndir, int nsplit, int R, int Cn) {
   CLSTM_GRID_STRIDE(e, (size_t)ndir * Cn) {
diff --git a/clstm_amd/csrc/runtime.inc b/clstm_amd/csrc/runtime.inc
--- a/clstm_amd/csrc/runtime.inc
+++ b/clstm_amd/csrc/runtime.inc
@@ -136,7 +136,8 @@
   PC_FWD_FUSED_WX = 6, PC_PEER_EXCHANGE = 7, PC_DW_X_EXTERNAL = 8, PC_BWD_C32 = 9, PC_PACKS_FOLLOW_UPDATE = 10, PC_BWD_X3 = 11,
   PC_REPLICA_CHECK = 12, PC_DW_BIAS_OUT = 13, PC_DW_DX_ONE_LAUNCH = 14, PC_MFMA_NOSAVE = 15, PC_MFMA_FWD = 16, PC_MFMA_BWD = 17,
   PC_MFMA_BWD_DW = 18, PC_INGEST_TAIL = 19, PC_INGEST_TAIL_USED = 20, PC_MFMA_ROUTED = 21 ,
-  PC_LINE_NOSAVE = 22, PC_FUSED_NOSAVE = 23, PC_PEER_TWO_PHASE = 24, PC_NORMALIZED = 25, PC_XD_PROLOGUE = 26, PC_XD_PRODUCERS = 27, PC_SCORE = 28, PC_BEAM = 29, PC_COUNT
+  PC_LINE_NOSAVE = 22, PC_FUSED_NOSAVE = 23, PC_PEER_TWO_PHASE = 24, PC_NORMALIZED = 25, PC_XD_PROLOGUE = 26, PC_XD_PRODUCERS = 27, PC_SCORE = 28, PC_BEAM = 29,
+  PC_REDUCE_ROLE = 30 , PC_COUNT
 };
 static long long g_path_count[PC_COUNT];
 struct StorePlain {
@@ -250,13 +251,14 @@
     else CLSTM_LAUNCH((lstm_bwd_xd_kernel<N, K, 2>), dim3(bs, a.ndir), dim3(nthreads), smem, s, a, x);
   });
 }
-static void launch_lstm_bwd_dw(int nk4, int ku, const LstmSeqArgs& a, const GemmDwArgs& g, int terms, int nrec, unsigned ngemm, int nthreads, hipStream_t s) {
+static void launch_lstm_bwd_dw(int nk4, int ku, const LstmSeqArgs& a, const GemmDwArgs& g, int terms, int nrec, unsigned ngemm, int nthreads, hipStream_t s,
+                               const DwLastRole& role = DwLastRole{}) {
   narrow_dispatch<NCAP_DW>(nk4, ku, [&](auto c) {
     constexpr int N = decltype(c)::NK4, K = decltype(c)::KU;
     const size_t smem = (2 * 16 * (size_t)lstm_qstride(N) + 4) * sizeof(float);
-    if (terms >= 3) CLSTM_LAUNCH((lstm_bwd_dw_kernel<N, K, 3>), dim3(nrec + ngemm), dim3(nthreads), smem, s, a, g, nrec);
-    else if (terms) CLSTM_LAUNCH((lstm_bwd_dw_kernel<N, K, 2>), dim3(nrec + ngemm), dim3(nthreads), smem, s, a, g, nrec);
-    else CLSTM_LAUNCH((lstm_bwd_dw_kernel<N, K, 0>), dim3(nrec + ngemm), dim3(nthreads), smem, s, a, g, nrec);
+    if (terms >= 3) CLSTM_LAUNCH((lstm_bwd_dw_kernel<N, K, 3>), dim3(nrec + ngemm), dim3(nthreads), smem, s, a, g, nrec, role);
+    else if (terms) CLSTM_LAUNCH((lstm_bwd_dw_kernel<N, K, 2>), dim3(nrec + ngemm), dim3(nthreads), smem, s, a, g, nrec, role);
+    else CLSTM_LAUNCH((lstm_bwd_dw_kernel<N, K, 0>), dim3(nrec + ngemm), dim3(nthreads), smem, s, a, g, nrec, role);
   });
 }
 static void launch_gemm_dw(const GemmDwArgs& g, int terms, unsigned nblk, hipStream_t s) {
diff --git a/clstm_amd/csrc/step.inc b/clstm_amd/csrc/step.inc
--- a/clstm_amd/csrc/step.inc
+++ b/clstm_amd/csrc/step.inc
@@ -69,26 +69,28 @@
   }
   n.forward();
   net_ctc_launch(n, ctc);
-  PassLeft left = n.backward(n.step_plan(next.given(), ticket));
+  PassLeft left = n.backward(n.step_plan(next.given() ? next.T : nullptr, next.bs, ticket));
   if (left.deferred.armed) {
     bool tail = !(n.L.size() == 1 && !n.L[0].wide && !left.packs_follow_update);
+    IngestTail t{};
     if (tail) {
       try {
         n.set_batch(next.T, next.bs);
         CtcMetaCopy meta;
         net_ctc(n, ctc, next, nullptr, &meta, false);
-        const IngestTail t = ingest_tail(n, next.x, meta);
-        n.launch_deferred_reduce(left.deferred, &t);
-        if (t.lo_src) { n.ring.commit(g_stream); n.lo_pending = false; }
-        if (t.aux_src) ctc.ring.commit(g_stream);
-        n.src0_ready = true;
-        n.next.remember(next);
+        t = ingest_tail(n, next.x, meta);
       } catch (...) {
         n.next.valid = false;
         tail = false;
       }
     }
-    if (!tail) n.launch_deferred_reduce(left.deferred, nullptr);
+    n.launch_deferred_reduce(left.deferred, tail ? &t : nullptr);
+    if (tail) {
+      if (t.lo_src) { n.ring.commit(g_stream); n.lo_pending = false; }
+      if (t.aux_src) ctc.ring.commit(g_stream);
+      n.src0_ready = true;
+      n.next.remember(next);
+    }
   }
   n.update(left);
   if (ticket) {
```

After: 231,900. About the same (-0.4%).
